# cyrillefavreau/Sol-R

Hardware: AMD Instinct MI355X
Metric: Mrays/s @1920x1080, 3-bounce Cornell (higher is better)
Workload: dtype f32; 1 GPU; cornell 1920x1080, 3 bounces + shadow rays, 75 boxes / 29 primitives, one GPU, whole frame; rays_per_frame=6518779, closest_hit_walks_rank0=3506171, lane_nodes=206382796, lane_prim_tests=37557299, wave_nodes=3396811, wave_prim_tests=626627, wave_walks=106204, cost_ordered_launch_rank0=True, frames_in_flight=3, setup_frames_before_warmup=48, frames_delivered=9105, order_free_nodes=43, short_ray_lists=1, gather=none (one GPU), strips=equal rows, parallelism=tile1

## Files before the change

sol-r_amd/csrc/engine.h:

```cpp
#ifndef SOLR_ENGINE_H
#define SOLR_ENGINE_H

#include <hip/hip_runtime.h>

#include <atomic>
#include <chrono>
#include <cstdio>
#include <cstdlib>
#include <cstring>
#include <string>
#include <vector>

#include "../../include/solr_hip.h"
#include "renderer.h"
#include "lists_device.h"
#include "list_builders.h"

namespace solreng
{
struct HostProfile
{
    const bool on = getenv("SOLR_HIP_HOST_PROFILE") != nullptr;
    struct Entry
    {
        const char *name;
        double seconds;
        long calls;
    } entries[16] = {};
    int used = 0;
    Entry *find(const char *name)
    {
        for (int i = 0; i < used; ++i)
            if (entries[i].name == name)
                return &entries[i];
        if (used < 16)
        {
            entries[used].name = name;
            return &entries[used++];
        }
        return nullptr;
    }
    void report()
    {
        if (!on)
            return;
        for (int i = 0; i < used; ++i)
            fprintf(stderr, "solr_hip host: %-34s %9.3f us per call over %ld calls\n", entries[i].name,
                    1e6 * entries[i].seconds / (entries[i].calls ? entries[i].calls : 1), entries[i].calls);
        used = 0;
    }
    ~HostProfile() { report(); }
};
extern HostProfile gHostProfile;
struct HostSpan
{
    const char *name;
    std::chrono::steady_clock::time_point t0;
    explicit HostSpan(const char *n) : name(n)
    {
        if (gHostProfile.on)
            t0 = std::chrono::steady_clock::now();
    }
    ~HostSpan()
    {
        if (!gHostProfile.on)
            return;
        if (HostProfile::Entry *e = gHostProfile.find(name))
        {
            e->seconds += std::chrono::duration<double>(std::chrono::steady_clock::now() - t0).count();
            e->calls++;
        }
    }
};

struct PhaseTimer
{
    const bool on = getenv("SOLR_HIP_DEBUG_TIMING") != nullptr;
    std::chrono::steady_clock::time_point last = std::chrono::steady_clock::now();
    void mark(const char *what)
    {
        if (!on)
            return;
        const auto now = std::chrono::steady_clock::now();
        fprintf(stderr, "solr_hip: %-28s %8.2f ms\n", what, std::chrono::duration<double, std::milli>(now - last).count());
        last = now;
    }
};

struct DeviceBuffer
{
    void *ptr = nullptr;
    size_t bytes = 0;
};
inline void release(DeviceBuffer &b)
{
    if (b.ptr)
        (void)hipFree(b.ptr);
    b.ptr = nullptr;
    b.bytes = 0;
}

const int MAX_FLIGHTS = 4;
struct Flight
{
    hipStream_t stream = nullptr;
    DeviceBuffer pp, ids;
    DeviceBuffer image[2];
    int side = 0;
    int copy[2] = {-1, -1};
    DeviceBuffer deepStack;
    DeviceBuffer haloAbove, haloBelow, haloSendTop, haloSendBottom;

    DeviceBuffer &shown() { return image[side]; }
    void forgetCopies()
    {
        copy[0] = copy[1] = -1;
        side = 0;
        solreng::release(image[1]);
    }
    void release()
    {
        for (DeviceBuffer *b : {&pp, &ids, &image[0], &deepStack, &haloAbove, &haloBelow, &haloSendTop, &haloSendBottom})
            solreng::release(*b);
        forgetCopies();
    }
};
struct SharedRing
{
    std::atomic<long> done[64][MAX_FLIGHTS + 2];
    std::atomic<long> consumed;
    long frameBytes, imageStride;
};
struct ImageRing
{
    static const int IMAGE_RING = MAX_FLIGHTS + 2;
    BitmapBuffer *pinnedImage[IMAGE_RING] = {};
    size_t pinnedBytes = 0;
    static const long TICKET_PERIOD = ((long)0x7fffffff / IMAGE_RING / IMAGE_RING - 1) * IMAGE_RING;
    static int ticketOf(long serial, int slot) { return (int)((serial % TICKET_PERIOD) * IMAGE_RING + slot); }
    long imageSerial = 0;
    long slotSerial[IMAGE_RING] = {};
    long shareSeq = 0;
    long slotShareSeq[IMAGE_RING] = {};
    long lastWaitedSeq = 0;
    long sharePublished[IMAGE_RING] = {};
    struct SharedRing *sharedRing = nullptr;
    size_t sharedBytes = 0;
    std::string sharedName;
    int shareRank = 0, shareWorld = 0;
    bool slotOfStrips[IMAGE_RING] = {};
    long lastHandedOut = 0;
    bool copyOnRenderStream = false;
    void release();
};
extern ImageRing gImageRing;
struct CopyLane
{
    hipStream_t stream = nullptr;
    hipEvent_t frameRendered = nullptr;
    hipEvent_t imageDone[ImageRing::IMAGE_RING] = {};
    void release();
};
struct ImageStreaming
{
    int next = 0;
    bool ids = false;
    bool valid = false;
    const void *bitmap = nullptr;
    unsigned serial = 0;
    long key[3] = {0, 0, 0};
    DeviceBuffer counters;
    StreamPlan plan = {};
    int bands = 0;
    unsigned *hostWords = nullptr;
    hipEvent_t rendered = nullptr;
    long delivered = 0;
    int support = -1;
    void release();
};
const int SORT_PERIOD = 64;

struct TileSchedule
{
    int mode = 1;
    DeviceBuffer cost, costSnapshot;
    DeviceBuffer order[2];
    int orderBuffer = 0;
    hipEvent_t orderEvent = nullptr;
    bool orderWait[MAX_FLIGHTS] = {};
    unsigned *hostStats = nullptr;
    unsigned *hostStatsDev = nullptr;
    long key[6] = {0, 0, 0, 0, 0, 0};
    int frames = 0;
    bool reorder = false;
    bool orderValid = false;
    BandCuts orderCuts = {};
    void reset()
    {
        frames = 0;
        reorder = false;
        orderValid = false;
    }
    void release();
};

enum Variant
{
    VARIANT_AUTOMATIC = 0,
    VARIANT_EXACT_LIST = 3,
    VARIANT_ALL_FEATURES = 4,
    VARIANT_NO_GROUPING = 5,
    VARIANT_NO_ORDER_FREE = 6,
    VARIANT_STACK_IN_LDS = 7,
    VARIANT_REFERENCE_LEAVES = 8,
    VARIANT_AO_FIXED_STRIDE = 9,
    VARIANT_NAN_DEEP_STACK = 10,
    VARIANT_UNSORTED_LISTS = 12,
    VARIANT_NO_BAND_WORDS = 13,
    VARIANT_ZERO_STREAM_COUNTERS = 14,
    VARIANT_NO_LAMP_CUTOFF = 15,
    VARIANT_ALL_TRIPS = 16
};

struct NodeList
{
    int copies, lists;
    explicit NodeList(int copies_ = 1, int lists_ = 1) : copies(copies_), lists(lists_) {}
    std::vector<float4> rows;
    std::vector<int> start, origin;
    int nb = 0;
    unsigned offRows = 0, offLeaf = 0;
    unsigned offStart = 0;
    int ordered = 0;
    bool tight = false;
    std::vector<int> refitLevels;

    void reset() { *this = NodeList(copies, lists); }
    unsigned nodes() const { return (unsigned)lists * (unsigned)nb; }
    unsigned rowsOf(int list) const { return solrdev::listRows(offRows, (unsigned)nb, (unsigned)list); }
    unsigned offThin() const { return solrdev::listThin(offRows, nodes()); }
    unsigned offSorted() const { return solrdev::listSorted(offRows, nodes()); }
    unsigned layRows(unsigned row)
    {
        offRows = row;
        return row + (unsigned)copies * solrdev::listCopyRows(nodes());
    }
    unsigned layStart(unsigned row)
    {
        offStart = row * 4;
        return row + (nodes() + 3u) / 4u;
    }
    unsigned layLeaf(unsigned row)
    {
        row = (row + 3u) & ~3u;
        offLeaf = row;
        return row + 4u * nodes() + 4u;
    }
};


struct Arena
{
    DeviceBuffer geometry;
    unsigned offPrims = 0, offLights = 0;
    unsigned rowsFixed = 0;
    bool geometryDirty = true;
    bool deviceAhead = false;
    void layOutAgain() { geometryDirty = true; }
};
struct OrderFreeState
{
    int freeCountdown = 0;
    bool freeHostValid = true;
    bool freeDirty = false;
    SolrDeviceLists freeStage;
    bool freeStale = false;
    bool sortedFree = false;
    void dropStage(bool originToo)
    {
        if (freeStage.rows)
            (void)hipFree(freeStage.rows);
        if (freeStage.start)
            (void)hipFree(freeStage.start);
        freeStage.rows = nullptr;
        freeStage.start = nullptr;
        if (originToo && freeStage.origin)
        {
            (void)hipFree(freeStage.origin);
            freeStage.origin = nullptr;
        }
    }
};
struct Rotation
{
    DeviceBuffer movable, refitPlan;
    DeviceBuffer enclosesFlag;
    int nbMovable = -1;
    bool refitReady = false;
    bool refitPlanPending = false;
    bool exactStale = false;
    float exactStaleViewDistance = 0.f;
    int nbDeviceRotations = 0;
};
struct Scene
{
    NodeList exact = NodeList(1, 1), walk = NodeList(2, 1), orderFree = NodeList(3, solrdev::ORDER_FREE_LISTS);
    std::vector<float4> hostPrims;
    int nbPrimitives = 0;
    DeviceBuffer lamps;
    int nbLamps = 0;
    int nested = 1;
    bool walkEncloses = false;
    OrderFreeState lists;
    Rotation rotation;
    Arena arena;

    void newGeometry(int nested_, bool walkEncloses_, int freeCountdown_)
    {
        nested = nested_;
        walkEncloses = walkEncloses_;
        rotation.refitReady = false;
        rotation.exactStale = false;
        rotation.refitPlanPending = true;
        rotation.nbMovable = -1;
        arena.deviceAhead = false;
        orderFree.reset();
        lists.freeCountdown = freeCountdown_;
        lists.freeHostValid = true;
        lists.freeDirty = false;
        lists.dropStage(true);
        lists.freeStale = false;
    }
    bool orderFreeDue() { return lists.freeCountdown > 0 && --lists.freeCountdown == 0; }
    void orderFreeAskAgain() { lists.freeCountdown = 1; }
    void orderFreeBuilt(const NodeList &built, bool stayed, bool fromArena)
    {
        orderFree = built;
        lists.freeHostValid = !stayed;
        lists.freeStale = false;
        rotation.refitReady = false;
        rotation.refitPlanPending = true;
        if (stayed && fromArena)
            lists.freeDirty = true;
        else
            arena.layOutAgain();
    }
    void listsAppended()
    {
        lists.dropStage(false);
        lists.freeDirty = false;
    }
    void arenaFlushed()
    {
        arena.geometryDirty = false;
        lists.freeDirty = false;
    }
    void hostListsPulled()
    {
        lists.freeHostValid = true;
        lists.dropStage(true);
    }
    void hostImagesPulled() { arena.deviceAhead = false; }
    void rotationQueued(bool listsFollow, float viewDistance)
    {
        if (!listsFollow)
            lists.freeStale = orderFree.nb > 0;
        rotation.exactStale = true;
        rotation.exactStaleViewDistance = viewDistance;
    }
    void exactRefitted() { rotation.exactStale = false; }
    void rotationServed(bool walkHolds, bool landed)
    {
        walkEncloses = walkHolds;
        if (landed)
        {
            arena.deviceAhead = true;
            ++rotation.nbDeviceRotations;
        }
    }
    void release()
    {
        lists.dropStage(true);
        for (DeviceBuffer *b : {&arena.geometry, &lamps, &rotation.movable, &rotation.refitPlan, &rotation.enclosesFlag})
            solreng::release(*b);
        *this = Scene();
    }
};
struct Lights
{
    std::vector<float4> hostLights;
    int nbLights = 0;
};
struct TextureUse
{
    int material;
    long texels;
    long offsets[7];
};
struct Materials
{
    DeviceBuffer table;
    unsigned offMatCold = 0;
    int nbMaterials = 0;
    std::vector<int> materialTags;
    std::vector<float> materialAverage;
    std::vector<TextureUse> textureUses;
    void release()
    {
        solreng::release(table);
        *this = Materials();
    }
};
struct Textures
{
    DeviceBuffer atlas;
    size_t atlasBytes = 0;
    bool textureTablesChecked = false;
    void release()
    {
        solreng::release(atlas);
        *this = Textures();
    }
};
struct Randoms
{
    DeviceBuffer values;
    long nbRandoms = 0;
    float randomsReach = 0.f;
    void release()
    {
        solreng::release(values);
        *this = Randoms();
    }
};
struct SceneFacts
{
    bool primsContained = false;
    bool opaqueShadows = false;
    bool plainPlanes = false;
    float sceneExtent = 1.f;
    int sceneFeatures = F_ALL & ~F_FULL;
};
struct KernelTimer
{
    unsigned timingTick = 0;
    std::vector<std::pair<hipEvent_t, hipEvent_t>> events;
    double timedMs = 0.0;
    int timedLaunches = 0;
    std::vector<float> kernelSamples, intervalSamples;
};
struct WalkRecording
{
    DeviceBuffer walkRecords, walkVisits;
    bool recordNext = false;
    bool recorded = false;
    unsigned recordGrid = 0;
    size_t recordLds = 0;
    int recordVariant = -1;
    bool recordDeep = false;
    SceneArgs recordScene = {};
    void release()
    {
        solreng::release(walkRecords);
        solreng::release(walkVisits);
        *this = WalkRecording();
    }
};

struct Engine
{
    bool initialized = false;
    int device = 0;
    int errorCode = 0;
    std::string errorText;

    int variant = VARIANT_AUTOMATIC;
    bool grouping = true;
    int shortRayListsMode = -1;
    int flights = 1;
    bool tileClocks = false;
    int timing = 0;

    Scene scene;
    Lights lights;
    Materials materials;
    Textures textures;
    Randoms randoms;
    SceneFacts facts;

    DeviceBuffer counters, tileClock;
    DeviceBuffer haloGivenAbove, haloGivenBelow;
    int haloSuppliedAbove = 0, haloSuppliedBelow = 0;
    int haloWanted = -1;
    Flight flight[MAX_FLIGHTS];
    bool ownStream = false;
    bool callerStreams = false;
    int current = 0;
    unsigned frameSerial = 0;
    TileSchedule sched;
    unsigned lastSerial = 0;
    int nbTilesTimed = 0;
    void *boundBitmap = nullptr;
    int width = 0, height = 0;
    int firstRow = 0, nbRows = -1;
    int allocW = 0, allocRows = 0;

    KernelTimer timer;
    WalkRecording recording;

    CopyLane copyLane;
    ImageStreaming streaming;
    int tileCheckedX = 0, tileCheckedTiles = 0, tileCheckedShift = 0;
    unsigned tileCheckedMagic = 0;
    int lastMask = -1;
    int lastFrame[6] = {-1, -1, 0, 0, 0, 0};
};

extern Engine gFirst;
extern Engine *gEngines[SOLR_MAX_GPU_COUNT];
extern int gDevices;
extern int gRequested;
extern Engine *gCurrent;
#define g (*gCurrent)
template <class F>
void onEveryDevice(F &&f)
{
    for (int d = 0; d < gDevices; ++d)
    {
        gCurrent = gEngines[d];
        if (gDevices > 1)
            (void)hipSetDevice(g.device);
        f(d);
    }
    gCurrent = &gFirst;
    if (gDevices > 1)
        (void)hipSetDevice(g.device);
}

inline int activeFlights()
{
    if (g.flights < 2 || !(g.ownStream || g.callerStreams))
        return 1;
    int n = 1;
    while (n < g.flights && n < MAX_FLIGHTS && g.flight[n].stream)
        ++n;
    return n;
}
inline bool twoFlights() { return activeFlights() > 1; }
inline hipStream_t sceneStream() { return g.flight[0].stream; }
inline void quiesce()
{
    for (int f = 1; f < MAX_FLIGHTS; ++f)
        if (g.flight[f].stream)
            (void)hipStreamSynchronize(g.flight[f].stream);
    if (g.flight[0].stream)
        (void)hipStreamSynchronize(g.flight[0].stream);
    if (g.copyLane.stream)
        (void)hipStreamSynchronize(g.copyLane.stream);
}

inline void setError(int code, const char *what, const char *file, int line)
{
    if (g.errorCode != 0)
        return;
    g.errorCode = code;
    char buf[512];
    snprintf(buf, sizeof(buf), "%s (%s:%d)", what, file, line);
    g.errorText = buf;
    fprintf(stderr, "solr_hip: error %d: %s\n", code, buf);
    const char *fatal = getenv("SOLR_HIP_FATAL");
    if (fatal && fatal[0] == '1')
        exit(EXIT_FAILURE);
}

#define HIPCHECK(expr)                                                                                           \
    do                                                                                                           \
    {                                                                                                            \
        hipError_t e_ = (expr);                                                                                  \
        if (e_ != hipSuccess)                                                                                    \
        {                                                                                                        \
            std::string m_ = std::string(#expr) + ": " + hipGetErrorString(e_);                                  \
            setError((int)e_, m_.c_str(), __FILE__, __LINE__);                                                   \
        }                                                                                                        \
    } while (0)

#define ARGCHECK(cond, msg)                                                                                      \
    do                                                                                                           \
    {                                                                                                            \
        if (!(cond))                                                                                             \
            setError(-1, msg, __FILE__, __LINE__);                                                               \
    } while (0)

inline bool ok()
{
    return g.errorCode == 0;
}

inline bool ready(const char *who)
{
    if (!ok())
        return false;
    if (!g.initialized)
    {
        setError(-1, (std::string(who) + ": initialize_scene has not been called").c_str(), __FILE__, __LINE__);
        return false;
    }
    return true;
}

inline void reserve(DeviceBuffer &b, size_t bytes)
{
    if (bytes < 16)
        bytes = 16;
    if (b.ptr && b.bytes >= bytes)
        return;
    release(b);
    HIPCHECK(hipMalloc(&b.ptr, bytes));
    if (ok())
        b.bytes = bytes;
}

template <class T>
void upload(DeviceBuffer &b, const std::vector<T> &host)
{
    reserve(b, host.size() * sizeof(T));
    if (ok() && !host.empty())
    {
        HIPCHECK(hipMemcpyAsync(b.ptr, host.data(), host.size() * sizeof(T), hipMemcpyHostToDevice, sceneStream()));
        HIPCHECK(hipStreamSynchronize(sceneStream()));
    }
}

inline int stripRows()
{
    return g.nbRows >= 0 ? g.nbRows : g.height;
}


void h2dSceneOne(BoundingBox *boundingBoxes, int nbActiveBoxes, Primitive *primitives, int nbPrimitives, Lamp *lamps, int nbLamps);
void h2dMaterialsOne(Material *materials, int nbActiveMaterials);
void h2dRandomsOne(float *randoms);
void h2dRandomsSizedOne(const float *randoms, long count);
void h2dTexturesOne(int activeTextures, TextureInfo *textureInfos);
void h2dLightInformationOne(LightInformation *lightInformation, int lightInformationSize);
void setMovableOne(const unsigned char *flags, int nbPrimitives);
void checkTextureTables();
void maybeBuildOrderFreeLists();
void flushGeometry();
void pullGeometry();
void ensureHostFreeLists();
void buildLeafRecords();
bool listEnclosesInArena(const NodeList &list);
ListKnobs listKnobs();
PruneDecider pruneDecider();
bool orderFreeListsUsable();
bool lampCutoffUsable();
bool shortRayListsChoice();
SceneArgs prepareScene(const SceneInfo &sceneInfo, bool exactNodes);
bool deepNodeList(const SceneArgs &S);
bool canRotateOne(const float center[3], const float cosAngles[3], const float sinAngles[3], float viewDistance);
int rotatePrimitivesOne(const float center[3], const float cosAngles[3], const float sinAngles[3], float viewDistance);
void refreshExactList();
void allocateFrame();
int neededFeatures(const SceneInfo &sceneInfo, bool full);
void renderImpl(const SceneInfo &sceneInfo, const vec4i &objects, const PostProcessingInfo &ppInfo, const float origin[3],
                const float direction[3], const float angles[4], bool counting, unsigned long long counts[8]);
void collectEvents();
void d2hBitmapOne(const SceneInfo &sceneInfo, BitmapBuffer *bitmap, PrimitiveXYIdBuffer *primitivesXYIds, bool wait);
void d2hBitmapWait();
void releaseCopies();
bool imageStreamingCuts(int tileRows, int firstRow[SOLR_STREAM_BANDS_MAX + 1], int *bands, bool withIds);
bool armImageStreaming(FrameArgs &F, int tileRows, hipStream_t stream, bool withIds);
void markStreamedFrame(hipStream_t stream);
void ensureCopyStream();
bool ensureImageRing();
int nextTicket(int *slot);
bool haveCommunicator();
bool communicatorUp();
int agreedHaloRows(const PostProcessingInfo &ppInfo);
void exchangeDepthHalo(int flight, hipStream_t stream, const PixelRecord *pp, int W, int firstRow, int nbRows, int frameRows,
                       int wanted, DepthHalo *halo);
bool shareRandoms();

struct HaloDebt
{
    bool owed = false;
    int wanted = 0, width = 0, frameRows = 0;
    ~HaloDebt()
    {
        if (owed)
            exchangeDepthHalo(g.current, g.flight[g.current].stream, nullptr, width, 0, 0, frameRows, wanted, nullptr);
    }
};
void launchPostProcess(const SceneInfo &sceneInfo, const PostProcessingInfo &ppInfo, int flight, hipStream_t stream, int firstRow,
                       int nbRows, unsigned char *bitmap, HaloDebt &debt);
}

namespace solrpost
{
void defaultConversion(hipStream_t stream, const SceneInfo &si, int nbPixels, const PixelRecord *pp, unsigned char *bitmap);
void ambientOcclusion(hipStream_t stream, const SceneInfo &si, const PostProcessingInfo &ppi, int nbRows, const PixelRecord *pp,
                      const float *randoms, long nbRandoms, unsigned char *bitmap, const DepthHalo &halo, int firstRow,
                      float randomsReach, bool heavyFirst);
void depthOfField(hipStream_t stream, const SceneInfo &si, const PostProcessingInfo &ppi, int nbRows, const PixelRecord *pp,
                  const float *randoms, long nbRandoms, unsigned char *bitmap);
void radiosity(hipStream_t stream, const SceneInfo &si, const PostProcessingInfo &ppi, int nbRows, const PixelRecord *pp,
               const int4 *ids, const float *randoms, long nbRandoms, unsigned char *bitmap);
void filter(hipStream_t stream, const SceneInfo &si, const PostProcessingInfo &ppi, int nbRows, const PixelRecord *pp,
            unsigned char *bitmap);
void cartoon(hipStream_t stream, const SceneInfo &si, const PostProcessingInfo &ppi, int nbRows, const PixelRecord *pp,
             unsigned char *bitmap);
void orderTiles(hipStream_t stream, const unsigned *cost, unsigned *snapshot, unsigned *order, int nbTiles,
                volatile unsigned *hostStats, int flights, const BandCuts &cuts);
void packDepthRows(hipStream_t stream, const PixelRecord *pp, int W, int row0, int n, float *out);
}

#endif
```

sol-r_amd/csrc/list_builders.cpp:

```cpp
#include "list_builders.h"

#include <algorithm>
#include <cmath>

namespace solreng
{
int validateNesting(const BoundingBox *boxes, int n)
{
    std::vector<int> ends;
    for (int i = 0; i < n; ++i)
    {
        const int skip = boxes[i].indexForNextBox.x;
        if (skip < 1 || (long)i + skip > n)
            return 0;
        while (!ends.empty() && ends.back() <= i)
            ends.pop_back();
        const int end = i + skip;
        if (!ends.empty() && end > ends.back())
            return 0;
        ends.push_back(end);
    }
    return 1;
}

int collapseChains(const std::vector<float4> &rows, const std::vector<int> &start, bool nested, std::vector<float4> &outRows,
                   std::vector<int> &outStart, std::vector<int> &outOrigin, int *orderedExact, int *orderedWalk)
{
    const int n = (int)start.size();
    auto countOf = [&](int i) { return bitsi(rows[2 * i + 1].z); };
    auto skipOf = [&](int i) { return bitsi(rows[2 * i + 1].w); };
    std::vector<char> keep(n, 1);
    std::vector<int> newIndex((size_t)n + 1);
    newIndex[0] = 0;
    *orderedExact = 1;
    *orderedWalk = 1;
    for (int i = 0; i < n; ++i)
    {
        if (nested && countOf(i) == 0)
        {
            if (i + 1 < n)
            {
                if (skipOf(i) >= 2 && skipOf(i + 1) == skipOf(i) - 1 && memcmp(&rows[2 * i], &rows[2 * i + 2], 16) == 0 &&
                    memcmp(&rows[2 * i + 1], &rows[2 * i + 3], 8) == 0)
                    keep[i] = 0;
            }
            if (skipOf(i) == 1)
                keep[i] = 0;
        }
        const float lo[3] = {rows[2 * i].x, rows[2 * i].y, rows[2 * i].z}, hi[3] = {rows[2 * i + 1].x, rows[2 * i + 1].y, rows[2 * i].w};
        bool ordered = true;
        for (int k = 0; k < 3; ++k)
            ordered = ordered && (lo[k] <= hi[k]) && (fabsf(lo[k]) < 1.0e30f) && (fabsf(hi[k]) < 1.0e30f);
        if (!ordered)
        {
            *orderedExact = 0;
            if (keep[i])
                *orderedWalk = 0;
        }
        newIndex[(size_t)i + 1] = newIndex[i] + (keep[i] ? 1 : 0);
    }
    const int nc = newIndex[n];
    outRows.assign(2 * (size_t)nc, make_float4(0.f, 0.f, 0.f, 0.f));
    outStart.assign(nc, 0);
    outOrigin.assign(nc, 0);
    for (int i = 0; i < n; ++i)
        if (keep[i])
        {
            const int j = newIndex[i];
            outOrigin[j] = i;
            const int end = std::min(i + skipOf(i), n);
            outRows[2 * j] = rows[2 * i];
            outRows[2 * j + 1] = rows[2 * i + 1];
            outRows[2 * j + 1].w = bitsf(newIndex[end] - j);
            outStart[j] = start[i];
        }
    return nc;
}

int pruneInnerNodes(std::vector<float4> &rows, std::vector<int> &start, std::vector<int> &origin, int *nbPruned, double threshold,
                    const PruneDecider &decider)
{
    const int n = (int)start.size();
    *nbPruned = 0;
    if (n < 2 || !(threshold > 0.0))
        return n;
    auto skipOf = [&](int i) { return std::max(bitsi(rows[2 * i + 1].w), 1); };
    auto countOf = [&](int i) { return bitsi(rows[2 * i + 1].z); };
    auto lo = [&](int i, int k) { return k == 0 ? rows[2 * i].x : (k == 1 ? rows[2 * i].y : rows[2 * i].z); };
    auto hi = [&](int i, int k) { return k == 0 ? rows[2 * i + 1].x : (k == 1 ? rows[2 * i + 1].y : rows[2 * i].w); };
    auto areaOf = [&](int i) {
        const double x = (double)hi(i, 0) - lo(i, 0), y = (double)hi(i, 1) - lo(i, 1), z = (double)hi(i, 2) - lo(i, 2);
        return x * y + y * z + z * x;
    };
    std::vector<char> keep(n, 1);
    const int decided = decider ? decider(rows.data(), n, threshold, keep) : -1;
    if (decided >= 0)
        *nbPruned = decided;
    else
    {
        keep.assign(n, 1);
        std::vector<int> leaves;
        std::vector<int> leavesBefore(n + 1, 0);
        for (int i = 0; i < n; ++i)
        {
            leavesBefore[i + 1] = leavesBefore[i] + (countOf(i) > 0 ? 1 : 0);
            if (countOf(i) > 0)
                leaves.push_back(i);
        }
        struct Open
        {
            int node, end;
        };
        std::vector<Open> open;
        double sceneLo[3] = {1e300, 1e300, 1e300}, sceneHi[3] = {-1e300, -1e300, -1e300};
        for (int j = 0; j < n; j += skipOf(j))
            for (int k = 0; k < 3; ++k)
            {
                sceneLo[k] = std::min(sceneLo[k], (double)lo(j, k));
                sceneHi[k] = std::max(sceneHi[k], (double)hi(j, k));
            }
        const double sceneArea = (sceneHi[0] - sceneLo[0]) * (sceneHi[1] - sceneLo[1]) + (sceneHi[1] - sceneLo[1]) * (sceneHi[2] - sceneLo[2]) +
                                 (sceneHi[2] - sceneLo[2]) * (sceneHi[0] - sceneLo[0]);
        for (int i = 0; i < n; ++i)
        {
            while (!open.empty() && open.back().end <= i)
                open.pop_back();
            const int end = std::min(i + skipOf(i), n);
            if (countOf(i) == 0 && end > i + 1)
            {
                const int parentFrom = open.empty() ? 0 : open.back().node, parentTo = open.empty() ? n : open.back().end;
                const double parentArea = open.empty() ? sceneArea : areaOf(open.back().node);
                const double bySurface = parentArea > 0.0 ? std::min(1.0, areaOf(i) / parentArea) : 1.0;
                const int firstLeaf = leavesBefore[parentFrom], lastLeaf = leavesBefore[parentTo];
                const int stride = std::max(1, (lastLeaf - firstLeaf) / 4096);
                int sampled = 0, inside = 0;
                for (int q = firstLeaf; q < lastLeaf; q += stride)
                {
                    const int leaf = leaves[q];
                    bool in = true;
                    for (int k = 0; k < 3 && in; ++k)
                    {
                        const double c = 0.5 * ((double)lo(leaf, k) + hi(leaf, k));
                        in = c >= lo(i, k) && c <= hi(i, k);
                    }
                    ++sampled;
                    inside += in ? 1 : 0;
                }
                const double byOrigin = sampled ? (double)inside / sampled : 1.0;
                bool encloses = true;
                for (int j = i + 1; j < end && encloses; j += skipOf(j))
                    for (int k = 0; k < 3; ++k)
                        encloses = encloses && lo(j, k) >= lo(i, k) && hi(j, k) <= hi(i, k);
                if (encloses && (1.0 - std::max(bySurface, byOrigin)) * (end - i - 1) < threshold)
                {
                    keep[i] = 0;
                    ++*nbPruned;
                    continue;
                }
            }
            open.push_back({i, end});
        }
    }
    if (*nbPruned == 0)
        return n;
    std::vector<int> newIndex(n + 1, 0);
    for (int i = 0; i < n; ++i)
        newIndex[i + 1] = newIndex[i] + (keep[i] ? 1 : 0);
    const int m = newIndex[n];
    std::vector<float4> outRows(2 * (size_t)m);
    std::vector<int> outStart(m), outOrigin(m);
    for (int i = 0; i < n; ++i)
        if (keep[i])
        {
            const int j = newIndex[i];
            const int end = std::min(i + skipOf(i), n);
            outRows[2 * j] = rows[2 * i];
            outRows[2 * j + 1] = rows[2 * i + 1];
            outRows[2 * j + 1].w = bitsf(newIndex[end] - j);
            outStart[j] = start[i];
            outOrigin[j] = origin[i];
        }
    rows.swap(outRows);
    start.swap(outStart);
    origin.swap(outOrigin);
    return m;
}

int groupSiblings(std::vector<float4> &rows, std::vector<int> &start, std::vector<int> &origin, const ListKnobs &knobs)
{
    const int n = (int)start.size();
    auto skipOf = [&](int i) { return bitsi(rows[2 * i + 1].w); };
    struct Bounds
    {
        float lo[3], hi[3];
    };
    auto boundsOf = [&](int i) {
        Bounds b;
        b.lo[0] = rows[2 * i].x, b.lo[1] = rows[2 * i].y, b.lo[2] = rows[2 * i].z;
        b.hi[0] = rows[2 * i + 1].x, b.hi[1] = rows[2 * i + 1].y, b.hi[2] = rows[2 * i].w;
        return b;
    };
    auto merge = [](Bounds a, const Bounds &b) {
        for (int k = 0; k < 3; ++k)
        {
            a.lo[k] = std::min(a.lo[k], b.lo[k]);
            a.hi[k] = std::max(a.hi[k], b.hi[k]);
        }
        return a;
    };
    auto area = [](const Bounds &b) {
        const double x = (double)b.hi[0] - b.lo[0], y = (double)b.hi[1] - b.lo[1], z = (double)b.hi[2] - b.lo[2];
        return x * y + y * z + z * x;
    };
    std::vector<float4> outRows;
    std::vector<int> outStart, outOrigin;
    outRows.reserve(rows.size() + rows.size() / 2);
    outStart.reserve(start.size() + start.size() / 2);
    outOrigin.reserve(start.size() + start.size() / 2);

    std::vector<Bounds> suffix;
    auto splitPoint = [&](const std::vector<int> &sib, int from, int to) {
        const int count = to - from;
        suffix.resize((size_t)count);
        Bounds acc = boundsOf(sib[to - 1]);
        suffix[count - 1] = acc;
        for (int k = count - 2; k >= 0; --k)
        {
            acc = merge(acc, boundsOf(sib[from + k]));
            suffix[k] = acc;
        }
        Bounds left = boundsOf(sib[from]);
        double best = 1e300;
        int bestAt = from + count / 2;
        for (int k = 1; k < count; ++k)
        {
            const double cost = area(left) * k + area(suffix[k]) * (count - k);
            if (cost < best)
            {
                best = cost;
                bestAt = from + k;
            }
            left = merge(left, boundsOf(sib[from + k]));
        }
        return bestAt;
    };

    const int flatMax = std::max(1, knobs.groupFlat);
    struct Emit
    {
        std::function<void(const std::vector<int> &, int, int)> siblings;
        std::function<void(int)> node;
    } emit;
    emit.node = [&](int i) {
        const size_t at = outStart.size();
        outRows.push_back(rows[2 * i]);
        outRows.push_back(rows[2 * i + 1]);
        outStart.push_back(start[i]);
        outOrigin.push_back(origin[i]);
        const int end = std::min(i + skipOf(i), n);
        int few = 0;
        for (int j = i + 1; j < end && few <= flatMax; j += std::max(skipOf(j), 1))
            ++few;
        if (few > flatMax)
        {
            std::vector<int> children;
            for (int j = i + 1; j < end; j += std::max(skipOf(j), 1))
                children.push_back(j);
            emit.siblings(children, 0, (int)children.size());
        }
        else
            for (int j = i + 1; j < end;)
            {
                const int next = j + std::max(skipOf(j), 1);
                emit.node(j);
                j = next;
            }
        outRows[2 * at + 1].w = bitsf((int)(outStart.size() - at));
    };
    const int levels = std::min(4, std::max(1, knobs.groupLevels >= 0 ? knobs.groupLevels : (n <= 64 ? 3 : 2)));
    emit.siblings = [&](const std::vector<int> &sib, int from, int to) {
        if (to - from <= flatMax)
        {
            for (int k = from; k < to; ++k)
                emit.node(sib[k]);
            return;
        }
        {
            Bounds u = boundsOf(sib[from]);
            for (int k = from + 1; k < to; ++k)
                u = merge(u, boundsOf(sib[k]));
            const double limit = 0.5 * area(u);
            bool dominant = false;
            for (int k = from; k < to && !dominant; ++k)
                dominant = area(boundsOf(sib[k])) > limit;
            if (dominant)
            {
                int runStart = from;
                for (int k = from; k <= to; ++k)
                    if (k == to || area(boundsOf(sib[k])) > limit)
                    {
                        if (k > runStart)
                            emit.siblings(sib, runStart, k);
                        if (k < to)
                            emit.node(sib[k]);
                        runStart = k + 1;
                    }
                return;
            }
        }
        int parts[17];
        int np = 1;
        parts[0] = from;
        parts[1] = to;
        for (int level = 0; level < levels; ++level)
        {
            int next[17];
            int nn = 0;
            for (int q = 0; q < np; ++q)
            {
                next[nn++] = parts[q];
                if (parts[q + 1] - parts[q] > 2)
                    next[nn++] = splitPoint(sib, parts[q], parts[q + 1]);
            }
            next[nn] = to;
            np = nn;
            for (int q = 0; q <= np; ++q)
                parts[q] = next[q];
        }
        for (int q = 0; q < np; ++q)
        {
            const int a = parts[q], b = parts[q + 1];
            if (b - a == 1)
            {
                emit.node(sib[a]);
                continue;
            }
            Bounds u = boundsOf(sib[a]);
            for (int k = a + 1; k < b; ++k)
                u = merge(u, boundsOf(sib[k]));
            const size_t at = outStart.size();
            outRows.push_back(make_float4(u.lo[0], u.lo[1], u.lo[2], u.hi[2]));
            outRows.push_back(make_float4(u.hi[0], u.hi[1], bitsf(0), bitsf(1)));
            outStart.push_back(0);
            outOrigin.push_back(-1);
            emit.siblings(sib, a, b);
            outRows[2 * at + 1].w = bitsf((int)(outStart.size() - at));
        }
    };
    std::vector<int> top;
    for (int j = 0; j < n; j += std::max(skipOf(j), 1))
        top.push_back(j);
    emit.siblings(top, 0, (int)top.size());
    rows.swap(outRows);
    start.swap(outStart);
    origin.swap(outOrigin);
    return (int)start.size();
}

int buildWalkOrderList(std::vector<float4> &rows, std::vector<int> &start, std::vector<int> &origin, const ListKnobs &knobs,
                       const PruneDecider &decider, int *prunedBefore, int *prunedAfter, const std::function<void(const char *)> &mark)
{
    pruneInnerNodes(rows, start, origin, prunedBefore, knobs.pruneThreshold, decider);
    if (mark)
        mark("prune");
    groupSiblings(rows, start, origin, knobs);
    if (mark)
        mark("grouping");
    const int n = pruneInnerNodes(rows, start, origin, prunedAfter, knobs.pruneThreshold, decider);
    if (mark)
        mark("prune groups");
    return n;
}

int buildFreeOrderLists(const std::vector<float4> &rows, const std::vector<int> &start, const std::vector<int> &origin,
                        std::vector<float4> &outRows, std::vector<int> &outStart, std::vector<int> &outOrigin, int *nbPruned,
                        double threshold, const PruneDecider &decider)
{
    struct Leaf
    {
        float lo[3], hi[3];
        int node;
    };
    struct TreeNode
    {
        float lo[3], hi[3];
        int left, right, axis, leaf;
        bool keep;
    };
    const int n = (int)start.size();
    std::vector<Leaf> leaves;
    for (int i = 0; i < n; ++i)
        if (bitsi(rows[2 * i + 1].z) > 0)
        {
            Leaf l;
            l.lo[0] = rows[2 * i].x, l.lo[1] = rows[2 * i].y, l.lo[2] = rows[2 * i].z;
            l.hi[0] = rows[2 * i + 1].x, l.hi[1] = rows[2 * i + 1].y, l.hi[2] = rows[2 * i].w;
            l.node = i;
            leaves.push_back(l);
        }
    outRows.clear();
    outStart.clear();
    outOrigin.clear();
    *nbPruned = 0;
    if (leaves.size() < 2)
        return 0;
    auto area = [](const float *lo, const float *hi) {
        const double x = (double)hi[0] - lo[0], y = (double)hi[1] - lo[1], z = (double)hi[2] - lo[2];
        return x * y + y * z + z * x;
    };
    std::vector<TreeNode> tree;
    tree.reserve(2 * leaves.size());
    struct Range
    {
        int from, to, node;
    };
    std::vector<Range> todo;
    tree.push_back(TreeNode());
    todo.push_back({0, (int)leaves.size(), 0});
    while (!todo.empty())
    {
        const Range r = todo.back();
        todo.pop_back();
        const int count = r.to - r.from;
        TreeNode t;
        t.left = t.right = -1;
        t.axis = 0;
        t.leaf = -1;
        t.keep = true;
        if (count == 1)
        {
            for (int k = 0; k < 3; ++k)
                t.lo[k] = leaves[r.from].lo[k], t.hi[k] = leaves[r.from].hi[k];
            t.leaf = leaves[r.from].node;
            tree[r.node] = t;
            continue;
        }
        float clo[3] = {1e30f, 1e30f, 1e30f}, chi[3] = {-1e30f, -1e30f, -1e30f};
        for (int k = 0; k < 3; ++k)
            t.lo[k] = 1e30f, t.hi[k] = -1e30f;
        for (int q = r.from; q < r.to; ++q)
            for (int k = 0; k < 3; ++k)
            {
                t.lo[k] = std::min(t.lo[k], leaves[q].lo[k]);
                t.hi[k] = std::max(t.hi[k], leaves[q].hi[k]);
                const float c = 0.5f * (leaves[q].lo[k] + leaves[q].hi[k]);
                clo[k] = std::min(clo[k], c);
                chi[k] = std::max(chi[k], c);
            }
        for (int k = 0; k < 3; ++k)
            t.lo[k] += 0.f, t.hi[k] += 0.f;
        const int BINS = 16;
        int bestAxis = -1, bestBin = 0;
        double bestCost = 1e300;
        {
            int counts[3][BINS];
            float blo[3][BINS][3], bhi[3][BINS][3];
            float scale[3];
            for (int axis = 0; axis < 3; ++axis)
            {
                const float extent = chi[axis] - clo[axis];
                scale[axis] = extent > 0.f ? BINS / extent : 0.f;
                for (int b = 0; b < BINS; ++b)
                {
                    counts[axis][b] = 0;
                    for (int k = 0; k < 3; ++k)
                        blo[axis][b][k] = 1e30f, bhi[axis][b][k] = -1e30f;
                }
            }
            for (int q = r.from; q < r.to; ++q)
            {
                const Leaf &l = leaves[q];
                for (int axis = 0; axis < 3; ++axis)
                {
                    if (!(scale[axis] > 0.f))
                        continue;
                    const float c = 0.5f * (l.lo[axis] + l.hi[axis]);
                    const int b = std::min(BINS - 1, std::max(0, (int)((c - clo[axis]) * scale[axis])));
                    ++counts[axis][b];
                    float *lo3 = blo[axis][b], *hi3 = bhi[axis][b];
                    lo3[0] = std::min(lo3[0], l.lo[0]), lo3[1] = std::min(lo3[1], l.lo[1]), lo3[2] = std::min(lo3[2], l.lo[2]);
                    hi3[0] = std::max(hi3[0], l.hi[0]), hi3[1] = std::max(hi3[1], l.hi[1]), hi3[2] = std::max(hi3[2], l.hi[2]);
                }
            }
            for (int axis = 0; axis < 3; ++axis)
            {
                if (!(scale[axis] > 0.f))
                    continue;
                double rightArea[BINS];
                int rightCount[BINS];
                float rlo[3] = {1e30f, 1e30f, 1e30f}, rhi[3] = {-1e30f, -1e30f, -1e30f};
                int rc = 0;
                for (int b = BINS - 1; b > 0; --b)
                {
                    rc += counts[axis][b];
                    for (int k = 0; k < 3; ++k)
                    {
                        rlo[k] = std::min(rlo[k], blo[axis][b][k]);
                        rhi[k] = std::max(rhi[k], bhi[axis][b][k]);
                    }
                    rightCount[b] = rc;
                    rightArea[b] = rc ? area(rlo, rhi) : 0.0;
                }
                float llo[3] = {1e30f, 1e30f, 1e30f}, lhi[3] = {-1e30f, -1e30f, -1e30f};
                int lc = 0;
                for (int b = 0; b + 1 < BINS; ++b)
                {
                    lc += counts[axis][b];
                    for (int k = 0; k < 3; ++k)
                    {
                        llo[k] = std::min(llo[k], blo[axis][b][k]);
                        lhi[k] = std::max(lhi[k], bhi[axis][b][k]);
                    }
                    if (lc == 0 || rightCount[b + 1] == 0)
                        continue;
                    const double cost = area(llo, lhi) * lc + rightArea[b + 1] * rightCount[b + 1];
                    if (cost < bestCost)
                    {
                        bestCost = cost;
                        bestAxis = axis;
                        bestBin = b;
                    }
                }
            }
        }
        int mid;
        if (bestAxis < 0)
            mid = r.from + count / 2;
        else
        {
            const float scale = BINS / (chi[bestAxis] - clo[bestAxis]);
            const float origin = clo[bestAxis];
            const int axis = bestAxis, bin = bestBin;
            mid = (int)(std::stable_partition(leaves.begin() + r.from, leaves.begin() + r.to,
                                       [&](const Leaf &l) {
                                           const float c = 0.5f * (l.lo[axis] + l.hi[axis]);
                                           return std::min(BINS - 1, std::max(0, (int)((c - origin) * scale))) <= bin;
                                       }) -
                        leaves.begin());
            if (mid == r.from || mid == r.to)
                mid = r.from + count / 2;
            t.axis = bestAxis;
        }
        t.left = (int)tree.size();
        t.right = t.left + 1;
        tree.push_back(TreeNode());
        tree.push_back(TreeNode());
        tree[r.node] = t;
        todo.push_back({r.from, mid, t.left});
        todo.push_back({mid, r.to, t.right});
    }

    auto flatten = [&](int octant, std::vector<float4> &fr, std::vector<int> &fs, std::vector<int> *which,
                       std::vector<int> *from) {
        struct Visit
        {
            int node, slot;
        };
        std::vector<Visit> stack;
        stack.push_back({0, -1});
        while (!stack.empty())
        {
            const Visit v = stack.back();
            stack.pop_back();
            if (v.slot >= 0)
            {
                fr[2 * v.slot + 1].w = bitsf((int)fs.size() - v.slot);
                continue;
            }
            const TreeNode &t = tree[v.node];
            if (t.leaf >= 0)
            {
                fr.push_back(rows[2 * t.leaf]);
                float4 second = rows[2 * t.leaf + 1];
                second.w = bitsf(1);
                fr.push_back(second);
                fs.push_back(start[t.leaf]);
                if (which)
                    which->push_back(v.node);
                if (from)
                    from->push_back(origin[t.leaf]);
                continue;
            }
            if (t.keep)
            {
                const int slot = (int)fs.size();
                fr.push_back(make_float4(t.lo[0], t.lo[1], t.lo[2], t.hi[2]));
                fr.push_back(make_float4(t.hi[0], t.hi[1], bitsf(0), bitsf(1)));
                fs.push_back(0);
                if (which)
                    which->push_back(v.node);
                if (from)
                    from->push_back(-1);
                stack.push_back({0, slot});
            }
            const bool highFirst = (octant >> t.axis) & 1;
            stack.push_back({highFirst ? t.left : t.right, -1});
            stack.push_back({highFirst ? t.right : t.left, -1});
        }
    };
    {
        std::vector<float4> fr;
        std::vector<int> fs, which;
        flatten(0, fr, fs, &which, nullptr);
        std::vector<int> survivors(which);
        pruneInnerNodes(fr, fs, survivors, nbPruned, threshold, decider);
        std::vector<char> kept(tree.size(), 0);
        for (int t : survivors)
            kept[t] = 1;
        for (size_t t = 0; t < tree.size(); ++t)
            if (tree[t].leaf < 0)
                tree[t].keep = kept[t] != 0;
    }
    std::vector<int> size(tree.size(), 0);
    for (int t = (int)tree.size() - 1; t >= 0; --t)
        size[t] = tree[t].leaf >= 0 ? 1 : (tree[t].keep ? 1 : 0) + size[tree[t].left] + size[tree[t].right];
    const int count = size[0];
    outRows.assign(16 * (size_t)count, make_float4(0.f, 0.f, 0.f, 0.f));
    outStart.assign(8 * (size_t)count, 0);
    outOrigin.assign(8 * (size_t)count, -1);
    struct Place
    {
        int node, at;
    };
    std::vector<Place> stack;
    for (int octant = 0; octant < 8; ++octant)
    {
        float4 *fr = outRows.data() + 2 * (size_t)octant * count;
        int *fs = outStart.data() + (size_t)octant * count, *fo = outOrigin.data() + (size_t)octant * count;
        stack.clear();
        stack.push_back({0, 0});
        while (!stack.empty())
        {
            const Place v = stack.back();
            stack.pop_back();
            const TreeNode &t = tree[v.node];
            if (t.leaf >= 0)
            {
                fr[2 * v.at] = rows[2 * t.leaf];
                float4 second = rows[2 * t.leaf + 1];
                second.w = bitsf(1);
                fr[2 * v.at + 1] = second;
                fs[v.at] = start[t.leaf];
                fo[v.at] = origin[t.leaf];
                continue;
            }
            int at = v.at;
            if (t.keep)
            {
                fr[2 * at] = make_float4(t.lo[0], t.lo[1], t.lo[2], t.hi[2]);
                fr[2 * at + 1] = make_float4(t.hi[0], t.hi[1], bitsf(0), bitsf(size[v.node]));
                ++at;
            }
            const bool highFirst = (octant >> t.axis) & 1;
            const int first = highFirst ? t.right : t.left, second = highFirst ? t.left : t.right;
            stack.push_back({second, at + size[first]});
            stack.push_back({first, at});
        }
    }
    return count;
}

bool listEnclosesOnHost(const std::vector<float4> &rows, const std::vector<int> &start, const std::vector<float4> &prims)
{
    const int n = (int)start.size();
    if (rows.size() < 2 * (size_t)n)
        return false;
    auto skipOf = [&](int i) { return std::max(bitsi(rows[2 * i + 1].w), 1); };
    bool encloses = true;
    for (int i = 0; i < n && encloses; ++i)
    {
        const int end = std::min(i + skipOf(i), n);
        if (bitsi(rows[2 * i + 1].z) > 0 || end <= i + 1)
            continue;
        for (int j = i + 1; j < end && encloses; j += skipOf(j))
            encloses = rows[2 * j].x >= rows[2 * i].x && rows[2 * j].y >= rows[2 * i].y && rows[2 * j].z >= rows[2 * i].z &&
                       rows[2 * j + 1].x <= rows[2 * i + 1].x && rows[2 * j + 1].y <= rows[2 * i + 1].y &&
                       rows[2 * j].w <= rows[2 * i].w;
    }
    const size_t nbPrims = prims.size() / LB_PRIM_ROWS;
    for (int i = 0; i < n && encloses; ++i)
    {
        const int count = bitsi(rows[2 * i + 1].z);
        for (int k = 0; k < count && encloses; ++k)
        {
            const size_t pi = (size_t)start[i] + k;
            if (start[i] < 0 || pi >= nbPrims)
            {
                encloses = false;
                break;
            }
            const float4 *r = &prims[LB_PRIM_ROWS * pi];
            const int type = bitsi(r[LB_ROW_P0_TYPE].w) & LB_PRIM_TYPE_MASK;
            float lo[3] = {r[LB_ROW_P0_TYPE].x, r[LB_ROW_P0_TYPE].y, r[LB_ROW_P0_TYPE].z};
            float hi[3] = {lo[0], lo[1], lo[2]};
            auto add = [&](const float4 &v) {
                lo[0] = std::min(lo[0], v.x), lo[1] = std::min(lo[1], v.y), lo[2] = std::min(lo[2], v.z);
                hi[0] = std::max(hi[0], v.x), hi[1] = std::max(hi[1], v.y), hi[2] = std::max(hi[2], v.z);
            };
            float grow[3] = {r[LB_ROW_SIZE_MAT].x, r[LB_ROW_SIZE_MAT].y, r[LB_ROW_SIZE_MAT].z};
            if (type == ptTriangle)
            {
                add(r[LB_ROW_P1_INDEX]);
                add(r[LB_ROW_P2]);
                grow[0] = grow[1] = grow[2] = 0.f;
            }
            else if (type == ptCylinder)
            {
                add(r[LB_ROW_P1_INDEX]);
                grow[1] = grow[2] = grow[0];
            }
            else if (type == ptSphere)
                grow[1] = grow[2] = grow[0];
            auto slack = [&](int k) { return 4.f * 1.1920929e-7f * std::max(std::max(fabsf(lo[k]), fabsf(hi[k])), fabsf(grow[k])); };
            const float ex = slack(0), ey = slack(1), ez = slack(2);
            encloses = rows[2 * i].x <= lo[0] - fabsf(grow[0]) + ex && rows[2 * i].y <= lo[1] - fabsf(grow[1]) + ey &&
                       rows[2 * i].z <= lo[2] - fabsf(grow[2]) + ez && rows[2 * i + 1].x >= hi[0] + fabsf(grow[0]) - ex &&
                       rows[2 * i + 1].y >= hi[1] + fabsf(grow[1]) - ey && rows[2 * i].w >= hi[2] + fabsf(grow[2]) - ez;
        }
    }
    return encloses;
}

void planRefit(const std::vector<float4> &exact, const std::vector<float4> &walk, const std::vector<int> &origin,
               const std::vector<float4> &free, const std::vector<int> &freeOrigin, std::vector<int> &plan,
               std::vector<int> &exactLevels, std::vector<int> &walkLevels, std::vector<int> &freeLevels)
{
    plan.clear();
    exactLevels.clear();
    walkLevels.clear();
    freeLevels.clear();

    auto heights = [](const std::vector<float4> &rows, std::vector<int> &height) {
        const int n = (int)(rows.size() / 2);
        height.assign(n, 0);
        std::vector<int> parent(n, -1), stack;
        for (int i = 0; i < n; ++i)
        {
            while (!stack.empty() && i >= stack.back() + std::max(bitsi(rows[2 * stack.back() + 1].w), 1))
                stack.pop_back();
            parent[i] = stack.empty() ? -1 : stack.back();
            stack.push_back(i);
        }
        int top = 0;
        for (int i = n - 1; i >= 0; --i)
        {
            if (parent[i] >= 0)
                height[parent[i]] = std::max(height[parent[i]], height[i] + 1);
            top = std::max(top, height[i]);
        }
        return n ? top + 1 : 0;
    };
    auto byHeight = [&](const std::vector<int> &height, int nbHeights, std::vector<int> &levels, auto entry) {
        std::vector<std::vector<int>> bucket((size_t)nbHeights);
        for (int i = 0; i < (int)height.size(); ++i)
        {
            const long e = entry(i);
            if (e != -1)
                bucket[(size_t)height[i]].push_back((int)e);
        }
        for (const std::vector<int> &b : bucket)
            if (!b.empty())
            {
                levels.push_back((int)plan.size());
                levels.push_back((int)b.size());
                plan.insert(plan.end(), b.begin(), b.end());
            }
    };
    std::vector<int> height;
    int nbHeights = heights(exact, height);
    byHeight(height, nbHeights, exactLevels, [](int i) { return i != 0 ? (long)i : -1L; });
    nbHeights = heights(walk, height);
    byHeight(height, nbHeights, walkLevels, [&](int j) {
        if (origin[j] == 0)
            return -1L;
        return origin[j] < 0 ? (long)(j | (int)0x80000000) : (long)j;
    });
    if (!free.empty())
    {
        nbHeights = heights(free, height);
        byHeight(height, nbHeights, freeLevels, [&](int j) {
            if (freeOrigin[j] == 0)
                return -1L;
            return freeOrigin[j] < 0 ? (long)(j | (int)0x80000000) : (long)j;
        });
    }
    if (plan.empty())
        plan.push_back(0);
}
}
```

sol-r_amd/csrc/list_builders.h:

```cpp
#ifndef SOLR_LIST_BUILDERS_H
#define SOLR_LIST_BUILDERS_H

#include <hip/hip_vector_types.h>

#include <cstring>
#include <functional>
#include <vector>

#include "../../include/solr_types.h"

namespace solreng
{
inline int bitsi(float v)
{
    int i;
    memcpy(&i, &v, sizeof(i));
    return i;
}
inline float bitsf(int v)
{
    float f;
    memcpy(&f, &v, 4);
    return f;
}

enum ListBuilderPrimRow
{
    LB_ROW_P0_TYPE = 0,
    LB_ROW_SIZE_MAT = 1,
    LB_ROW_P1_INDEX = 2,
    LB_ROW_P2 = 3,
    LB_PRIM_ROWS = 8,
    LB_PRIM_TYPE_MASK = 0xff
};

struct ListKnobs
{
    double pruneThreshold = 1.0;
    int groupFlat = 4;
    int groupLevels = -1;
};

typedef std::function<int(const float4 *rows, int n, double threshold, std::vector<char> &keep)> PruneDecider;

int validateNesting(const BoundingBox *boxes, int n);
int collapseChains(const std::vector<float4> &rows, const std::vector<int> &start, bool nested, std::vector<float4> &outRows,
                   std::vector<int> &outStart, std::vector<int> &outOrigin, int *orderedExact, int *orderedWalk);
int pruneInnerNodes(std::vector<float4> &rows, std::vector<int> &start, std::vector<int> &origin, int *nbPruned, double threshold,
                    const PruneDecider &decider = nullptr);
int groupSiblings(std::vector<float4> &rows, std::vector<int> &start, std::vector<int> &origin, const ListKnobs &knobs);
int buildWalkOrderList(std::vector<float4> &rows, std::vector<int> &start, std::vector<int> &origin, const ListKnobs &knobs,
                       const PruneDecider &decider, int *prunedBefore, int *prunedAfter,
                       const std::function<void(const char *)> &mark = nullptr);
int buildFreeOrderLists(const std::vector<float4> &rows, const std::vector<int> &start, const std::vector<int> &origin,
                        std::vector<float4> &outRows, std::vector<int> &outStart, std::vector<int> &outOrigin, int *nbPruned,
                        double threshold, const PruneDecider &decider = nullptr);
bool listEnclosesOnHost(const std::vector<float4> &rows, const std::vector<int> &start, const std::vector<float4> &prims);
void planRefit(const std::vector<float4> &exact, const std::vector<float4> &walk, const std::vector<int> &origin,
               const std::vector<float4> &free, const std::vector<int> &freeOrigin, std::vector<int> &plan,
               std::vector<int> &exactLevels, std::vector<int> &walkLevels, std::vector<int> &freeLevels);
}

#endif
```

sol-r_amd/csrc/lists_device.h:

```cpp
#pragma once
#include <hip/hip_runtime.h>

#include <vector>

struct SolrDeviceLists
{
    float4 *rows = nullptr;
    int *start = nullptr;
    int *origin = nullptr;
};

int solrBuildOrderFreeListsOnDevice(const float4 *rows, const int *start, const int *origin, int n, double threshold,
                                    int *nbPruned, hipStream_t stream, SolrDeviceLists *stay);

int solrPruneDecisionsOnDevice(const float4 *rows, int n, double threshold, std::vector<char> &keep, hipStream_t stream);
```

sol-r_amd/csrc/solr_arena.hip:

```cpp
#include <hip/hip_runtime.h>

#include <cmath>

#include "../../include/solr_hip.h"
#include "rt_device.h"

using namespace solrdev;

#include "renderer.h"
#include "engine.h"

using namespace solreng;

namespace solreng
{
__global__ __launch_bounds__(256) void k_buildLeafRecords(float4 *__restrict__ arena, unsigned offNodes, unsigned offStart,
                                                         unsigned offPrims, unsigned offLeaf, int nbNodes)
{
    const int i = blockIdx.x * blockDim.x + threadIdx.x;
    if (i >= nbNodes)
        return;
    float4 r0 = make_float4(0.f, 0.f, 0.f, 0.f), r1 = r0, r2 = r0, r3 = r0;
    const int nb = __float_as_int(arena[offNodes + 2u * (unsigned)i + 1u].z);
    if (nb > 0)
    {
        const int start = ((const int *)arena)[offStart + (unsigned)i];
        const float4 *prim = arena + offPrims + 8u * (unsigned)start;
        r0 = prim[ROW_P0_TYPE];
        r1 = prim[ROW_SIZE_MAT];
        r2 = prim[ROW_P1_INDEX];
        r3 = prim[ROW_P2];
        if (planeClass(__float_as_int(r0.w) & PRIM_TYPE_MASK))
        {
            const float4 n0 = prim[ROW_N0];
            r2 = make_float4(n0.x, n0.y, n0.z, r2.w);
            r3 = make_float4(r3.w, 0.f, 0.f, 0.f);
        }
        r3.w = __int_as_float(start);
    }
    float4 *out = arena + offLeaf + 4u * (unsigned)i;
    out[0] = r0;
    out[1] = r1;
    out[2] = r2;
    out[3] = r3;
}

__global__ __launch_bounds__(256) void k_tightenLeaves(float4 *__restrict__ arena, unsigned offNodes, unsigned offTight,
                                                      unsigned offStart, unsigned offPrims, int nbNodes, float margin)
{
    const int i = blockIdx.x * blockDim.x + threadIdx.x;
    if (i >= nbNodes)
        return;
    float4 row0 = arena[offNodes + 2u * (unsigned)i], row1 = arena[offNodes + 2u * (unsigned)i + 1u];
    const int nb = __float_as_int(row1.z);
    if (nb > 0)
    {
        const int start = ((const int *)arena)[offStart + (unsigned)i];
        float lx = INFINITY, ly = INFINITY, lz = INFINITY, hx = -INFINITY, hy = -INFINITY, hz = -INFINITY;
        bool plain = true;
        for (int k = 0; k < nb && plain; ++k)
        {
            const float4 *prim = arena + offPrims + 8u * (unsigned)(start + k);
            const float4 p = prim[ROW_P0_TYPE], s = prim[ROW_SIZE_MAT];
            const int kind = (__float_as_int(p.w) >> PRIM_KIND_SHIFT) & 15;
            plain = kind == KIND_PLANE_XY || kind == KIND_PLANE_YZ || kind == KIND_PLANE_XZ;
            const float ex = kind == KIND_PLANE_YZ ? margin : fabsf(s.x) + margin;
            const float ey = kind == KIND_PLANE_XZ ? margin : fabsf(s.y) + margin;
            const float ez = kind == KIND_PLANE_XY ? margin : fabsf(s.z) + margin;
            lx = fminf(lx, p.x - ex), hx = fmaxf(hx, p.x + ex);
            ly = fminf(ly, p.y - ey), hy = fmaxf(hy, p.y + ey);
            lz = fminf(lz, p.z - ez), hz = fmaxf(hz, p.z + ez);
        }
        plain = plain && lx <= hx && ly <= hy && lz <= hz && fabsf(lx) < 3.0e38f && fabsf(hx) < 3.0e38f && fabsf(ly) < 3.0e38f &&
                fabsf(hy) < 3.0e38f && fabsf(lz) < 3.0e38f && fabsf(hz) < 3.0e38f;
        if (plain)
        {
            const float nlx = fmaxf(row0.x, lx), nly = fmaxf(row0.y, ly), nlz = fmaxf(row0.z, lz);
            const float nhx = fminf(row1.x, hx), nhy = fminf(row1.y, hy), nhz = fminf(row0.w, hz);
            if (nlx <= nhx && nly <= nhy && nlz <= nhz)
            {
                row0 = make_float4(nlx, nly, nlz, nhz);
                row1 = make_float4(nhx, nhy, row1.z, row1.w);
            }
        }
    }
    arena[offTight + 2u * (unsigned)i] = row0;
    arena[offTight + 2u * (unsigned)i + 1u] = row1;
}

__global__ __launch_bounds__(256) void k_tightenInner(float4 *__restrict__ arena, unsigned offTight, int nbNodes, int listLength)
{
    const int i = blockIdx.x * blockDim.x + threadIdx.x;
    if (i >= nbNodes)
        return;
    const float4 row0 = arena[offTight + 2u * (unsigned)i], row1 = arena[offTight + 2u * (unsigned)i + 1u];
    const int nb = __float_as_int(row1.z), skip = __float_as_int(row1.w);
    if (nb > 0 || skip <= 1)
        return;
    const int listEnd = (i / listLength + 1) * listLength;
    const int end = min(i + skip, listEnd);
    float lx = INFINITY, ly = INFINITY, lz = INFINITY, hx = -INFINITY, hy = -INFINITY, hz = -INFINITY;
    for (int j = i + 1; j < end; ++j)
    {
        const float4 b = arena[offTight + 2u * (unsigned)j + 1u];
        if (__float_as_int(b.z) <= 0)
            continue;
        const float4 a = arena[offTight + 2u * (unsigned)j];
        lx = fminf(lx, a.x), ly = fminf(ly, a.y), lz = fminf(lz, a.z);
        hx = fmaxf(hx, b.x), hy = fmaxf(hy, b.y), hz = fmaxf(hz, a.w);
    }
    const float nlx = fmaxf(row0.x, lx), nly = fmaxf(row0.y, ly), nlz = fmaxf(row0.z, lz);
    const float nhx = fminf(row1.x, hx), nhy = fminf(row1.y, hy), nhz = fminf(row0.w, hz);
    if (!(nlx <= nhx && nly <= nhy && nlz <= nhz))
        return;
    arena[offTight + 2u * (unsigned)i] = make_float4(nlx, nly, nlz, nhz);
    arena[offTight + 2u * (unsigned)i + 1u] = make_float4(nhx, nhy, row1.z, row1.w);
}

__global__ __launch_bounds__(256) void k_listEncloses(const float4 *__restrict__ arena, unsigned offNodes, unsigned offStart,
                                                      unsigned offPrims, int nbNodes, int nbPrims, int *bad)
{
    const int i = blockIdx.x * blockDim.x + threadIdx.x;
    if (i >= nbNodes)
        return;
    const float4 a = arena[offNodes + 2u * (unsigned)i], b = arena[offNodes + 2u * (unsigned)i + 1u];
    const int count = __float_as_int(b.z);
    const int end = min(i + max(__float_as_int(b.w), 1), nbNodes);
    bool encloses = true;
    if (count <= 0)
    {
        for (int j = i + 1; j < end && encloses;)
        {
            const float4 ca = arena[offNodes + 2u * (unsigned)j], cb = arena[offNodes + 2u * (unsigned)j + 1u];
            encloses = ca.x >= a.x && ca.y >= a.y && ca.z >= a.z && cb.x <= b.x && cb.y <= b.y && ca.w <= a.w;
            j += max(__float_as_int(cb.w), 1);
        }
    }
    else
    {
        const int start = ((const int *)arena)[offStart + (unsigned)i];
        for (int k = 0; k < count && encloses; ++k)
        {
            const long long pi = (long long)start + k;
            if (start < 0 || pi >= nbPrims)
            {
                encloses = false;
                break;
            }
            const float4 *r = arena + offPrims + (size_t)PRIM_ROWS * (size_t)pi;
            const float4 p0 = r[ROW_P0_TYPE], size = r[ROW_SIZE_MAT];
            const int type = __float_as_int(p0.w) & PRIM_TYPE_MASK;
            float lo[3] = {p0.x, p0.y, p0.z}, hi[3] = {p0.x, p0.y, p0.z};
            auto add = [&](const float4 &v) {
                lo[0] = v.x < lo[0] ? v.x : lo[0], lo[1] = v.y < lo[1] ? v.y : lo[1], lo[2] = v.z < lo[2] ? v.z : lo[2];
                hi[0] = hi[0] < v.x ? v.x : hi[0], hi[1] = hi[1] < v.y ? v.y : hi[1], hi[2] = hi[2] < v.z ? v.z : hi[2];
            };
            float grow[3] = {size.x, size.y, size.z};
            if (type == ptTriangle)
            {
                add(r[ROW_P1_INDEX]);
                add(r[ROW_P2]);
                grow[0] = grow[1] = grow[2] = 0.f;
            }
            else if (type == ptCylinder)
            {
                add(r[ROW_P1_INDEX]);
                grow[1] = grow[2] = grow[0];
            }
            else if (type == ptSphere)
                grow[1] = grow[2] = grow[0];
            auto larger = [](float x, float y) { return x < y ? y : x; };
            auto slack = [&](int k) { return 4.f * 1.1920929e-7f * larger(larger(fabsf(lo[k]), fabsf(hi[k])), fabsf(grow[k])); };
            const float ex = slack(0), ey = slack(1), ez = slack(2);
            encloses = a.x <= lo[0] - fabsf(grow[0]) + ex && a.y <= lo[1] - fabsf(grow[1]) + ey && a.z <= lo[2] - fabsf(grow[2]) + ez &&
                       b.x >= hi[0] + fabsf(grow[0]) - ex && b.y >= hi[1] + fabsf(grow[1]) - ey && a.w >= hi[2] + fabsf(grow[2]) - ez;
        }
    }
    if (!encloses)
        *bad = 1;
}

void ensureHostFreeLists()
{
    if (g.scene.lists.freeHostValid || !ok())
        return;
    quiesce();
    NodeList &list = g.scene.orderFree;
    const size_t n = list.nodes();
    list.rows.resize(2 * n);
    list.start.resize(n);
    list.origin.resize(n);
    const bool staged = g.scene.lists.freeStage.rows != nullptr;
    const char *arena = (const char *)g.scene.arena.geometry.ptr;
    if (!staged && !arena)
    {
        setError(-1, "order-free lists neither staged nor in the arena", __FILE__, __LINE__);
        return;
    }
    HIPCHECK(hipMemcpy(list.rows.data(), staged ? (const void *)g.scene.lists.freeStage.rows : arena + (size_t)list.offRows * 16, 2 * n * 16,
                       hipMemcpyDeviceToHost));
    HIPCHECK(hipMemcpy(list.start.data(), staged ? (const void *)g.scene.lists.freeStage.start : arena + (size_t)list.offStart * 4, n * 4,
                       hipMemcpyDeviceToHost));
    if (g.scene.lists.freeStage.origin)
        HIPCHECK(hipMemcpy(list.origin.data(), g.scene.lists.freeStage.origin, n * 4, hipMemcpyDeviceToHost));
    if (ok())
    {
        g.scene.hostListsPulled();
    }
}

void pullGeometry()
{
    if (!g.scene.arena.deviceAhead || !g.scene.arena.geometry.ptr)
        return;
    refreshExactList();
    quiesce();
    auto get = [&](unsigned at, void *dst, size_t bytes) {
        if (bytes)
            HIPCHECK(hipMemcpy(dst, (const char *)g.scene.arena.geometry.ptr + (size_t)at * 16, bytes, hipMemcpyDeviceToHost));
    };
    for (NodeList *list : {&g.scene.exact, &g.scene.walk, &g.scene.orderFree})
        if (list != &g.scene.orderFree || g.scene.lists.freeHostValid)
            get(list->offRows, list->rows.data(), list->rows.size() * 16);
    get(g.scene.arena.offPrims, g.scene.hostPrims.data(), g.scene.hostPrims.size() * 16);
    g.scene.hostImagesPulled();
}

static bool tightenList(const NodeList &list)
{
    static const bool off = getenv("SOLR_HIP_NO_TIGHT_LEAVES") != nullptr;
    const int nbNodes = (int)list.nodes(), listLength = list.nb;
    if (off || !g.facts.plainPlanes || nbNodes <= 0 || listLength <= 0 || listLength > 65536 || !ok())
        return false;
    float4 *arena = (float4 *)g.scene.arena.geometry.ptr;
    const float margin = g.facts.sceneExtent * (1.f / 1024.f);
    const dim3 grid((unsigned)((nbNodes + 255) / 256));
    hipLaunchKernelGGL(k_tightenLeaves, grid, dim3(256), 0, sceneStream(), arena, list.offRows, list.offThin(), list.offStart, g.scene.arena.offPrims,
                       nbNodes, margin);
    hipLaunchKernelGGL(k_tightenInner, grid, dim3(256), 0, sceneStream(), arena, list.offThin(), nbNodes, listLength);
    HIPCHECK(hipGetLastError());
    return ok();
}

__global__ __launch_bounds__(256) void k_sortNodeBounds(float4 *__restrict__ arena, unsigned offBoxesFree, unsigned offSorted, int nb)
{
    const int i = blockIdx.x * blockDim.x + threadIdx.x;
    if (i > 8 * nb)
        return;
    float4 a = make_float4(0.f, 0.f, 0.f, 0.f), b = a;
    if (i < 8 * nb)
    {
        const int octant = i / nb;
        a = arena[offBoxesFree + 2u * (unsigned)i];
        b = arena[offBoxesFree + 2u * (unsigned)i + 1u];
        if (octant & 1)
        {
            const float t = a.x;
            a.x = b.x;
            b.x = t;
        }
        if (octant & 2)
        {
            const float t = a.y;
            a.y = b.y;
            b.y = t;
        }
        if (octant & 4)
        {
            const float t = a.z;
            a.z = a.w;
            a.w = t;
        }
        b.w = __int_as_float(__float_as_int(b.w) << 5);
    }
    arena[offSorted + 2u * (unsigned)i] = a;
    arena[offSorted + 2u * (unsigned)i + 1u] = b;
}

static bool sortFreeLists()
{
    static const bool off = getenv("SOLR_HIP_NO_SORTED_LISTS") != nullptr;
    const NodeList &list = g.scene.orderFree;
    if (off || list.nb <= 0 || !ok())
        return false;
    hipLaunchKernelGGL(k_sortNodeBounds, dim3((unsigned)((8 * list.nb + 1 + 255) / 256)), dim3(256), 0, sceneStream(),
                       (float4 *)g.scene.arena.geometry.ptr, list.offRows, list.offSorted(), list.nb);
    HIPCHECK(hipGetLastError());
    return ok();
}

static void deriveList(NodeList &list)
{
    const bool orderFree = &list == &g.scene.orderFree;
    const int n = (orderFree && g.scene.lists.freeStale) ? 0 : (int)list.nodes();
    if (n > 0)
        hipLaunchKernelGGL(k_buildLeafRecords, dim3((unsigned)((n + 255) / 256)), dim3(256), 0, sceneStream(), (float4 *)g.scene.arena.geometry.ptr,
                           list.offRows, list.offStart, g.scene.arena.offPrims, list.offLeaf, n);
    HIPCHECK(hipGetLastError());
    list.tight = list.copies > 1 && n > 0 && tightenList(list);
    if (orderFree)
        g.scene.lists.sortedFree = n > 0 && sortFreeLists();
}

void buildLeafRecords()
{
    if (!ok() || !g.scene.arena.geometry.ptr)
        return;
    for (NodeList *list : {&g.scene.exact, &g.scene.walk, &g.scene.orderFree})
        deriveList(*list);
    HIPCHECK(hipStreamSynchronize(sceneStream()));
}

static void copyStagedLists()
{
    const NodeList &list = g.scene.orderFree;
    char *arena = (char *)g.scene.arena.geometry.ptr;
    const SolrDeviceLists &stage = g.scene.lists.freeStage;
    HIPCHECK(hipMemcpyAsync(arena + (size_t)list.offRows * 16, stage.rows, (size_t)list.nodes() * 32, hipMemcpyDeviceToDevice, sceneStream()));
    HIPCHECK(hipMemcpyAsync(arena + (size_t)list.offStart * 4, stage.start, (size_t)list.nodes() * 4, hipMemcpyDeviceToDevice, sceneStream()));
}

static void appendFreeLists()
{
    const unsigned end = g.scene.orderFree.layLeaf(g.scene.orderFree.layStart(g.scene.orderFree.layRows(g.scene.arena.rowsFixed)));
    const size_t bytes = (size_t)end * 16, fixedBytes = (size_t)g.scene.arena.rowsFixed * 16;
    PhaseTimer phase;
    if (g.scene.arena.geometry.bytes < bytes)
    {
        DeviceBuffer larger;
        reserve(larger, bytes);
        if (!ok())
            return;
        HIPCHECK(hipMemcpyAsync(larger.ptr, g.scene.arena.geometry.ptr, fixedBytes, hipMemcpyDeviceToDevice, sceneStream()));
        HIPCHECK(hipStreamSynchronize(sceneStream()));
        release(g.scene.arena.geometry);
        g.scene.arena.geometry = larger;
    }
    HIPCHECK(hipMemsetAsync((char *)g.scene.arena.geometry.ptr + fixedBytes, 0, bytes - fixedBytes, sceneStream()));
    copyStagedLists();
    if (ok())
        deriveList(g.scene.orderFree);
    HIPCHECK(hipStreamSynchronize(sceneStream()));
    phase.mark("geometry: lists appended");
    if (ok())
        g.scene.listsAppended();
}

void flushGeometry()
{
    if (!g.scene.arena.geometryDirty)
    {
        if (g.scene.lists.freeDirty && g.scene.lists.freeStage.rows && g.scene.arena.geometry.ptr && g.scene.arena.rowsFixed > 0)
            appendFreeLists();
        else if (g.scene.lists.freeDirty)
            g.scene.arena.layOutAgain();
        if (!g.scene.arena.geometryDirty)
            return;
    }
    pullGeometry();
    if (!g.scene.lists.freeStage.rows)
        ensureHostFreeLists();
    unsigned row = g.scene.walk.layRows(g.scene.exact.layRows(0));
    row = (row + 3u) & ~3u;
    g.scene.arena.offPrims = row;
    row += (unsigned)g.scene.hostPrims.size();
    g.scene.arena.offLights = row;
    row += (unsigned)g.lights.hostLights.size();
    row = g.scene.walk.layStart(g.scene.exact.layStart(row));
    row = g.scene.walk.layLeaf(g.scene.exact.layLeaf(row));
    g.scene.arena.rowsFixed = row;
    row = g.scene.orderFree.layLeaf(g.scene.orderFree.layStart(g.scene.orderFree.layRows(row)));
    PhaseTimer phase;
    reserve(g.scene.arena.geometry, (size_t)std::max(row, 1u) * 16);
    if (!ok())
        return;
    HIPCHECK(hipMemsetAsync(g.scene.arena.geometry.ptr, 0, (size_t)std::max(row, 1u) * 16, sceneStream()));
    auto put = [&](unsigned at, const void *src, size_t bytes) {
        if (bytes && ok())
            HIPCHECK(hipMemcpyAsync((char *)g.scene.arena.geometry.ptr + (size_t)at * 16, src, bytes, hipMemcpyHostToDevice, sceneStream()));
    };
    for (const NodeList *list : {&g.scene.exact, &g.scene.walk, &g.scene.orderFree})
        if (list == &g.scene.orderFree && g.scene.lists.freeStage.rows)
        {
            if (ok())
                copyStagedLists();
        }
        else
        {
            put(list->offRows, list->rows.data(), list->rows.size() * 16);
            put(list->offStart / 4, list->start.data(), list->start.size() * 4);
        }
    put(g.scene.arena.offPrims, g.scene.hostPrims.data(), g.scene.hostPrims.size() * 16);
    put(g.scene.arena.offLights, g.lights.hostLights.data(), g.lights.hostLights.size() * 16);
    HIPCHECK(hipStreamSynchronize(sceneStream()));
    if (ok())
        g.scene.lists.dropStage(false);
    phase.mark("geometry: upload");
    buildLeafRecords();
    phase.mark("geometry: leaf records");
    if (ok())
        g.scene.arenaFlushed();
}

bool listEnclosesInArena(const NodeList &list)
{
    const int n = (int)list.nodes();
    HIPCHECK(hipSetDevice(g.device));
    reserve(g.scene.rotation.enclosesFlag, sizeof(int));
    if (!ok())
        return false;
    int found = 1;
    HIPCHECK(hipMemsetAsync(g.scene.rotation.enclosesFlag.ptr, 0, sizeof(int), sceneStream()));
    hipLaunchKernelGGL(k_listEncloses, dim3((unsigned)((n + 255) / 256)), dim3(256), 0, sceneStream(),
                       (const float4 *)g.scene.arena.geometry.ptr, list.offRows, list.offStart, g.scene.arena.offPrims, n,
                       (int)(g.scene.hostPrims.size() / PRIM_ROWS), (int *)g.scene.rotation.enclosesFlag.ptr);
    HIPCHECK(hipGetLastError());
    HIPCHECK(hipMemcpyAsync(&found, g.scene.rotation.enclosesFlag.ptr, sizeof(int), hipMemcpyDeviceToHost, sceneStream()));
    HIPCHECK(hipStreamSynchronize(sceneStream()));
    return ok() && found == 0;
}

ListKnobs listKnobs()
{
    ListKnobs knobs;
    if (const char *v = getenv("SOLR_HIP_PRUNE"))
        knobs.pruneThreshold = atof(v);
    if (const char *v = getenv("SOLR_HIP_GROUP_FLAT"))
        knobs.groupFlat = atoi(v);
    if (const char *v = getenv("SOLR_HIP_GROUP_LEVELS"))
        knobs.groupLevels = std::max(atoi(v), 0);
    return knobs;
}

PruneDecider pruneDecider()
{
    if (getenv("SOLR_HIP_LISTS_ON_HOST"))
        return nullptr;
    const hipStream_t stream = sceneStream();
    return [stream](const float4 *rows, int n, double threshold, std::vector<char> &keep) {
        return solrPruneDecisionsOnDevice(rows, n, threshold, keep, stream);
    };
}

void maybeBuildOrderFreeLists()
{
    if (!g.scene.orderFreeDue())
        return;
    if (!g.facts.primsContained)
    {
        g.scene.orderFreeAskAgain();
        return;
    }
    PhaseTimer phase;
    quiesce();
    pullGeometry();
    if (!ok())
        return;
    phase.mark("order-free: host images");
    const std::vector<float4> &rows = g.scene.exact.rows;
    const std::vector<int> &start = g.scene.exact.start;
    const int n = (int)start.size();
    if (n < 2 || rows.size() != 2 * (size_t)n || n > 16000000)
        return;
    const ListKnobs knobs = listKnobs();
    const bool onHost = getenv("SOLR_HIP_LISTS_ON_HOST") != nullptr;
    const bool fromArena = !g.scene.arena.geometryDirty && g.scene.arena.geometry.ptr != nullptr && !g.scene.rotation.exactStale &&
                           !g.scene.arena.deviceAhead && !onHost;
    const float4 *arena = (const float4 *)g.scene.arena.geometry.ptr;
    const bool encloses = fromArena ? listEnclosesInArena(g.scene.exact) : listEnclosesOnHost(rows, start, g.scene.hostPrims);
    if (!ok())
        return;
    if (!encloses)
    {
        if (getenv("SOLR_HIP_DEBUG_TREE"))
            fprintf(stderr, "solr_hip: no order-free lists: a node does not hold its children or primitives\n");
        return;
    }
    phase.mark("order-free: checks");
    std::vector<int> origin;
    auto ownOrigins = [&]() {
        origin.resize(n);
        for (int i = 0; i < n; ++i)
            origin[i] = i;
    };
    int prunedFree = 0;
    int count = -1;
    if (!onHost)
    {
        HIPCHECK(hipSetDevice(g.device));
        if (ok() && knobs.pruneThreshold > 0.0)
        {
            g.scene.lists.dropStage(true);
            if (fromArena)
                count = solrBuildOrderFreeListsOnDevice(arena + g.scene.exact.offRows, (const int *)arena + g.scene.exact.offStart, nullptr, n,
                                                        knobs.pruneThreshold, &prunedFree, sceneStream(), &g.scene.lists.freeStage);
            else
            {
                ownOrigins();
                count = solrBuildOrderFreeListsOnDevice(rows.data(), start.data(), origin.data(), n, knobs.pruneThreshold, &prunedFree,
                                                        sceneStream(), &g.scene.lists.freeStage);
            }
        }
    }
    const bool stayed = count > 0 && g.scene.lists.freeStage.rows != nullptr;
    NodeList built(g.scene.orderFree.copies, g.scene.orderFree.lists);
    if (count < 0)
    {
        if (origin.empty())
            ownOrigins();
        count = buildFreeOrderLists(rows, start, origin, built.rows, built.start, built.origin, &prunedFree, knobs.pruneThreshold,
                                    pruneDecider());
    }
    if (getenv("SOLR_HIP_DEBUG_TREE"))
        fprintf(stderr, "solr_hip: order-free lists: 8 x %d nodes (%d inner nodes that hardly cull left out)\n", count, prunedFree);
    if (count <= 0)
        return;
    phase.mark("order-free: tree, pruning, eight flattenings");
    built.nb = count;
    g.scene.orderFreeBuilt(built, stayed, fromArena);
}

bool orderFreeListsUsable()
{
    return g.scene.orderFree.nb > 0 && g.facts.primsContained && !g.scene.lists.freeStale && g.scene.nested && g.scene.walk.ordered &&
           g.variant != VARIANT_NO_ORDER_FREE;
}

bool lampCutoffUsable()
{
    return g.scene.walkEncloses && g.facts.primsContained && g.scene.nested && g.scene.walk.ordered && g.variant != VARIANT_NO_LAMP_CUTOFF;
}

static int tightListsFor(const SceneArgs &S, const SceneInfo &sceneInfo, bool exactNodes)
{
    if (exactNodes || g.variant == VARIANT_REFERENCE_LEAVES || !g.scene.walk.tight || !g.scene.walkEncloses || !sceneInfo.extendedGeometry)
        return 0;
    if (S.nbBoxesFree > 0 && !g.scene.orderFree.tight)
        return 0;
    return (sceneInfo.viewDistance > 0.f && sceneInfo.viewDistance <= 64.f * g.facts.sceneExtent) ? 1 : 0;
}

static bool sortedListsUsable(int nbBoxesFree)
{
    return nbBoxesFree > 0 && g.scene.lists.sortedFree && g.variant != VARIANT_UNSORTED_LISTS;
}

bool shortRayListsChoice()
{
    static const int fromEnv = getenv("SOLR_HIP_SHORT_RAY_LISTS") ? atoi(getenv("SOLR_HIP_SHORT_RAY_LISTS")) : -1;
    const int mode = g.shortRayListsMode >= 0 ? g.shortRayListsMode : fromEnv;
    return mode < 0 ? activeFlights() >= 2 : mode != 0;
}

static SceneArgs makeScene(bool exactNodes)
{
    const NodeList &list = exactNodes ? g.scene.exact : g.scene.walk;
    SceneArgs S;
    memset(&S, 0, sizeof(S));
    S.geometry = g.scene.arena.geometry.ptr;
    S.materials = g.materials.table.ptr;
    S.textures = g.textures.atlas.ptr;
    S.randoms = g.randoms.values.ptr;
    S.offBoxes = list.offRows;
    S.offBoxStart = list.offStart;
    S.offLeaf = list.offLeaf;
    S.offPrims = g.scene.arena.offPrims;
    S.offLights = g.scene.arena.offLights;
    S.offMatCold = g.materials.offMatCold;
    S.nbBoxes = list.nb;
    S.nbPrimitives = g.scene.nbPrimitives;
    S.nbLights = g.lights.nbLights;
    S.nbLamps = g.scene.nbLamps;
    S.nested = g.scene.nested;
    S.orderedBoxes = list.ordered;
    S.nbRandoms = g.randoms.values.ptr ? g.randoms.nbRandoms : 0;
    if (!exactNodes && orderFreeListsUsable())
    {
        S.offBoxesFree = g.scene.orderFree.offRows;
        S.offLeafFree = g.scene.orderFree.offLeaf;
        S.nbBoxesFree = g.scene.orderFree.nb;
        S.opaqueShadows = g.facts.opaqueShadows ? SHADOWS_OPAQUE : 0;
        S.shortRayLists = shortRayListsChoice() ? 1 : 0;
    }
    if (!exactNodes && lampCutoffUsable())
        S.opaqueShadows |= SHADOWS_LAMP_CUTOFF;
    if (g.variant == VARIANT_ALL_TRIPS)
        S.opaqueShadows |= SHADOWS_ALL_TRIPS;
    S.tightLists = 0;
    S.sortedLists = sortedListsUsable(S.nbBoxesFree) ? 1 : 0;
    return S;
}

SceneArgs prepareScene(const SceneInfo &sceneInfo, bool exactNodes)
{
    maybeBuildOrderFreeLists();
    flushGeometry();
    if (exactNodes)
        refreshExactList();
    if (!ok())
        return SceneArgs();
    SceneArgs S = makeScene(exactNodes);
    S.tightLists = tightListsFor(S, sceneInfo, exactNodes);
    return S;
}

bool deepNodeList(const SceneArgs &S)
{
    return S.nbBoxes > 1024;
}

}
```

sol-r_amd/csrc/solr_diag.hip:

```cpp
#include <hip/hip_runtime.h>
#include <dlfcn.h>
#include <fcntl.h>
#include <sched.h>
#include <sys/mman.h>
#include <sys/stat.h>
#include <unistd.h>

#include <atomic>

#include <cmath>
#include <cstdio>
#include <cstdlib>
#include <cstring>
#include <string>
#include <functional>
#include <chrono>
#include <vector>

#include "../../include/solr_hip.h"
#include "rt_device.h"
#include "device_pool.h"
#include "lists_device.h"

using namespace solrdev;

#include "renderer.h"
#include "engine.h"

using namespace solreng;

namespace solrprobe
{
int residentScene(const SceneInfo &sceneInfo, bool exactNodes, SceneArgs *S, int *features, int *deepList, hipStream_t *stream)
{
    if (!ready("solr_hip_probe"))
        return -1;
    quiesce();
    HIPCHECK(hipSetDevice(g.device));
    ARGCHECK(g.materials.table.ptr != nullptr, "solr_hip_probe: no materials uploaded");
    if (!ok())
        return -1;
    checkTextureTables();
    *S = prepareScene(sceneInfo, exactNodes);
    if (!ok())
        return -1;
    *features = neededFeatures(sceneInfo, false);
    *deepList = deepNodeList(*S);
    *stream = g.flight[0].stream;
    return 0;
}
void fail(int code, const char *what) { setError(code, what, __FILE__, __LINE__); }

int postProcess(const SceneInfo &sceneInfo, const PostProcessingInfo &ppInfo, const PostProcessingBuffer *frame,
                unsigned char *bitmapOut)
{
    if (!ready("solr_hip_probe_postprocess"))
        return -1;
    quiesce();
    HIPCHECK(hipSetDevice(g.device));
    ARGCHECK(frame != nullptr && bitmapOut != nullptr, "solr_hip_probe_postprocess: no buffer");
    ARGCHECK(sceneInfo.size.x > 0 && sceneInfo.size.y > 0, "solr_hip_probe_postprocess: empty image");
    ARGCHECK(g.nbRows < 0 && gDevices == 1, "solr_hip_probe_postprocess: whole frames of one device only");
    if (!ok())
        return -1;
    g.width = sceneInfo.size.x;
    g.height = sceneInfo.size.y;
    allocateFrame();
    if (!ok())
        return -1;
    const int flight = g.current;
    const hipStream_t stream = g.flight[flight].stream;
    const size_t pixels = (size_t)g.width * g.height;
    HIPCHECK(hipMemcpyAsync(g.flight[flight].pp.ptr, frame, pixels * sizeof(PostProcessingBuffer), hipMemcpyHostToDevice, stream));
    unsigned char *bitmap = (unsigned char *)g.flight[flight].shown().ptr;
    const bool neighbourhood = (ppInfo.type == ppe_ambientOcclusion || ppInfo.type == ppe_depthOfField ||
                                ppInfo.type == ppe_radiosity || ppInfo.type == ppe_filter || ppInfo.type == ppe_cartoon);
    if (neighbourhood)
    {
        HaloDebt nothingOwed;
        launchPostProcess(sceneInfo, ppInfo, flight, stream, 0, g.height, bitmap, nothingOwed);
    }
    else
    {
        solrpost::defaultConversion(stream, sceneInfo, (int)pixels, (const PixelRecord *)g.flight[flight].pp.ptr, bitmap);
        HIPCHECK(hipGetLastError());
    }
    HIPCHECK(hipMemcpyAsync(bitmapOut, bitmap, pixels * SOLR_COLOR_DEPTH, hipMemcpyDeviceToHost, stream));
    HIPCHECK(hipStreamSynchronize(stream));
    return ok() ? 0 : -1;
}

void lastFrame(int out[6])
{
    memcpy(out, g.lastFrame, sizeof(g.lastFrame));
}

int listCopy(int list, int what, void *out, int capacity)
{
    if (!ready("solr_hip_probe_list_copy"))
        return -1;
    ARGCHECK(list >= 0 && list <= 2 && what >= 0 && what <= 4, "solr_hip_probe_list_copy: no such list or copy");
    ARGCHECK(g.scene.arena.geometry.ptr != nullptr || g.scene.arena.geometryDirty, "solr_hip_probe_list_copy: no scene uploaded");
    if (!ok())
        return -1;
    HIPCHECK(hipSetDevice(g.device));
    flushGeometry();
    if (list == 1)
        refreshExactList();
    quiesce();
    if (!ok() || !g.scene.arena.geometry.ptr)
        return -1;
    const NodeList &L = list == 0 ? g.scene.walk : (list == 1 ? g.scene.exact : g.scene.orderFree);
    const unsigned nodes = (list == 2 && g.scene.lists.freeStale) ? 0u : L.nodes();
    size_t at = 0, count = 0, unit = 16;
    switch (what)
    {
    case 0:
        at = (size_t)L.offRows * 16, count = 2 * (size_t)nodes;
        break;
    case 1:
        at = (size_t)L.offThin() * 16, count = (L.copies > 1 && L.tight) ? 2 * (size_t)nodes : 0;
        break;
    case 2:
        at = (size_t)L.offSorted() * 16, count = (list == 2 && L.copies > 2 && g.scene.lists.sortedFree) ? 2 * (size_t)nodes + 2 : 0;
        break;
    case 3:
        at = (size_t)L.offLeaf * 16, count = 4 * (size_t)nodes;
        break;
    default:
        at = (size_t)L.offStart * 4, count = nodes, unit = 4;
        break;
    }
    if (nodes == 0)
        count = 0;
    if (!out)
        return (int)count;
    ARGCHECK(count <= (size_t)(capacity < 0 ? 0 : capacity), "solr_hip_probe_list_copy: capacity too small");
    ARGCHECK(at + count * unit <= g.scene.arena.geometry.bytes, "solr_hip_probe_list_copy: the copy lies outside the arena");
    if (!ok())
        return -1;
    if (count)
        HIPCHECK(hipMemcpy(out, (const char *)g.scene.arena.geometry.ptr + at, count * unit, hipMemcpyDeviceToHost));
    return ok() ? (int)count : -1;
}

int walkOffer(const SceneInfo &sceneInfo, bool exactNodes, int out[8])
{
    SceneArgs S;
    int features, deep;
    hipStream_t stream;
    if (residentScene(sceneInfo, exactNodes, &S, &features, &deep, &stream) != 0)
        return -1;
    const float margin = g.facts.sceneExtent * (1.f / 1024.f), extent = g.facts.sceneExtent;
    out[0] = S.tightLists, out[1] = S.sortedLists, out[2] = S.nbBoxesFree, out[3] = S.opaqueShadows, out[4] = S.shortRayLists;
    out[5] = S.nbBoxes;
    memcpy(&out[6], &margin, 4);
    memcpy(&out[7], &extent, 4);
    return 0;
}
}

extern "C" {
static unsigned long long walkLists[6];
void solr_hip_walk_bound_lists(unsigned long long out[6])
{
    if (out)
        memcpy(out, walkLists, sizeof(walkLists));
}

static int recordFrame(const SceneInfo *sceneInfo, const vec4i *objects, const PostProcessingInfo *postProcessingInfo,
                       const float origin[3], const float direction[3], const float angles[4], const char *who)
{
    quiesce();
    HIPCHECK(hipSetDevice(g.device));
    g.recording.recorded = false;
    g.recording.recordNext = true;
    if (!ok())
        return -1;
    renderImpl(*sceneInfo, *objects, *postProcessingInfo, origin, direction, angles, false, nullptr);
    g.recording.recordNext = false;
    HIPCHECK(hipStreamSynchronize(g.flight[g.current].stream));
    if (!ok() || !g.recording.recorded)
    {
        if (ok())
            setError(-1, "solr_hip_walk_bound: the frame was not recorded", __FILE__, __LINE__);
        return -1;
    }
    (void)who;
    return 0;
}

static int replayRecords(unsigned grid, size_t ldsBytes, int repeats, double ms[3], unsigned long long stats[4], bool lists)
{
    typedef WalkBoundFn BoundFn;
    ARGCHECK(g.recording.recordVariant >= 0 && g.recording.recordVariant < solrrows::LEAN_ROWS && g.recording.walkRecords.ptr && grid > 0 &&
                 (size_t)grid * SOLR_WALK_SLOT_BYTES <= g.recording.walkRecords.bytes,
             "solr_hip_walk_replay: no recorded frame, or more workgroups than its buffer holds");
    if (!ok())
        return -1;
    const int row = g.recording.recordVariant;
    const BoundFn fn = solrrows::walkBound(row, solrrows::ROWS[row].features | (g.recording.recordDeep ? F_DEEP : 0));
    ARGCHECK(fn != nullptr, "solr_hip_walk_bound: no replay instantiation for this row");
    if (!ok())
        return -1;
    reserve(g.recording.walkVisits, (size_t)grid * WAVE * sizeof(unsigned) + 64);
    hipEvent_t e0 = nullptr, e1 = nullptr;
    HIPCHECK(hipEventCreate(&e0));
    HIPCHECK(hipEventCreate(&e1));
    if (!ok())
        return -1;
    const hipStream_t stream = g.flight[g.current].stream;
    unsigned *visits = (unsigned *)g.recording.walkVisits.ptr;
    unsigned *skipped = visits + (size_t)grid * WAVE;
    double sum = 0.0, best = 1.0e30;
    repeats = repeats < 1 ? 1 : repeats;
    for (int i = 0; i < repeats + 2 && ok(); ++i)
    {
        HIPCHECK(hipMemsetAsync(skipped, 0, sizeof(unsigned), stream));
        HIPCHECK(hipEventRecord(e0, stream));
        hipLaunchKernelGGL(fn, dim3(grid), dim3(WAVE), ldsBytes, stream, g.recording.recordScene, (const char *)g.recording.walkRecords.ptr,
                           visits, skipped);
        HIPCHECK(hipGetLastError());
        HIPCHECK(hipEventRecord(e1, stream));
        HIPCHECK(hipEventSynchronize(e1));
        float t = 0.f;
        HIPCHECK(hipEventElapsedTime(&t, e0, e1));
        if (i >= 2)
        {
            sum += t;
            best = t < best ? t : best;
        }
    }
    if (ok() && stats)
    {
        std::vector<unsigned> v((size_t)grid * WAVE + 1);
        HIPCHECK(hipMemcpy(v.data(), visits, v.size() * sizeof(unsigned), hipMemcpyDeviceToHost));
        std::vector<int> heads((size_t)grid * 4);
        HIPCHECK(hipMemcpy2D(heads.data(), 16, g.recording.walkRecords.ptr, SOLR_WALK_SLOT_BYTES, 16, grid, hipMemcpyDeviceToHost));
        if (const char *dump = getenv("SOLR_HIP_WALK_BOUND_DUMP"))
        {
            if (FILE *f = fopen(dump, "wb"))
            {
                const unsigned n = grid;
                fwrite(&n, sizeof(n), 1, f);
                fwrite(v.data(), sizeof(unsigned), (size_t)n * WAVE, f);
                fwrite(heads.data(), sizeof(int), (size_t)n * 4, f);
                fclose(f);
            }
        }
        unsigned long long walks = 0, entries = 0;
        for (unsigned b = 0; b < grid; ++b)
            walks += (unsigned long long)heads[4 * (size_t)b];
        if (lists)
        {
            std::vector<int> kinds((size_t)grid * 4 * (SOLR_WALK_SLOTS + 1));
            HIPCHECK(hipMemcpy2D(kinds.data(), 16 * (SOLR_WALK_SLOTS + 1), g.recording.walkRecords.ptr, SOLR_WALK_SLOT_BYTES,
                                 16 * (SOLR_WALK_SLOTS + 1), grid, hipMemcpyDeviceToHost));
            for (int i = 0; i < 6; ++i)
                walkLists[i] = 0;
            for (unsigned b = 0; ok() && b < grid; ++b)
            {
                const int *slot = &kinds[(size_t)b * 4 * (SOLR_WALK_SLOTS + 1)];
                const int n = std::min(slot[0], (int)SOLR_WALK_SLOTS);
                for (int j = 0; j < n; ++j)
                {
                    const int kind = slot[4 * (1 + j)], freeList = slot[4 * (1 + j) + 1];
                    if (kind == WALK_CLOSEST || kind == WALK_SHADOW)
                        ++walkLists[2 * kind + (freeList ? 1 : 0)];
                    else
                        ++walkLists[4];
                }
                walkLists[5] += (unsigned long long)(slot[0] - n);
            }
        }
        for (size_t i = 0; i + 1 < v.size(); ++i)
            entries += v[i];
        stats[0] = walks;
        stats[1] = v.back();
        stats[2] = entries;
        stats[3] = grid;
    }
    if (ms)
    {
        ms[0] = 0.0;
        ms[1] = sum / repeats;
        ms[2] = best;
    }
    (void)hipEventDestroy(e0);
    (void)hipEventDestroy(e1);
    return ok() ? 0 : -1;
}

static bool keepWalkRecords = false;

int solr_hip_walk_bound(const SceneInfo *sceneInfo, const vec4i *objects, const PostProcessingInfo *postProcessingInfo,
                        const float origin[3], const float direction[3], const float angles[4], int repeats, double ms[3],
                        unsigned long long stats[4])
{
    if (!ready("solr_hip_walk_bound"))
        return -1;
    ARGCHECK(gDevices == 1, "solr_hip_walk_bound: a diagnostic of one engine; this process renders on several devices");
    if (!ok())
        return -1;
    if (recordFrame(sceneInfo, objects, postProcessingInfo, origin, direction, angles, "solr_hip_walk_bound") != 0)
        return -1;
    const int rc = replayRecords(g.recording.recordGrid, g.recording.recordLds, repeats, ms, stats, true);
    if (!keepWalkRecords)
    {
        release(g.recording.walkRecords);
        release(g.recording.walkVisits);
        g.recording.recorded = false;
    }
    return rc;
}

void solr_hip_walk_records_keep(int keep)
{
    keepWalkRecords = keep != 0;
}

int solr_hip_walk_records_info(unsigned long long info[4])
{
    if (!ready("solr_hip_walk_records_info") || !info)
        return -1;
    info[0] = g.recording.recorded ? g.recording.recordGrid : 0;
    info[1] = SOLR_WALK_SLOT_BYTES;
    info[2] = g.recording.recordLds;
    info[3] = SOLR_WALK_SLOTS;
    return 0;
}

int solr_hip_walk_records_copy(void *host, unsigned grid, int toDevice)
{
    if (!ready("solr_hip_walk_records_copy"))
        return -1;
    ARGCHECK(host && grid > 0 && g.recording.recorded, "solr_hip_walk_records_copy: no recorded frame");
    if (!ok())
        return -1;
    const size_t bytes = (size_t)grid * SOLR_WALK_SLOT_BYTES;
    HIPCHECK(hipSetDevice(g.device));
    if (toDevice)
    {
        reserve(g.recording.walkRecords, bytes);
        if (!ok())
            return -1;
        HIPCHECK(hipMemcpy(g.recording.walkRecords.ptr, host, bytes, hipMemcpyHostToDevice));
    }
    else
    {
        ARGCHECK(bytes <= g.recording.walkRecords.bytes, "solr_hip_walk_records_copy: more workgroups than were recorded");
        if (!ok())
            return -1;
        HIPCHECK(hipMemcpy(host, g.recording.walkRecords.ptr, bytes, hipMemcpyDeviceToHost));
    }
    return ok() ? 0 : -1;
}

int solr_hip_walk_replay(unsigned grid, long ldsBytes, int repeats, double ms[3], unsigned long long stats[4])
{
    if (!ready("solr_hip_walk_replay"))
        return -1;
    ARGCHECK(g.recording.recorded, "solr_hip_walk_replay: no recorded frame (solr_hip_walk_records_keep(1), then solr_hip_walk_bound)");
    if (!ok())
        return -1;
    HIPCHECK(hipSetDevice(g.device));
    return replayRecords(grid, ldsBytes < 0 ? g.recording.recordLds : (size_t)ldsBytes, repeats, ms, stats, false);
}

void solr_hip_walk_records_release(void)
{
    release(g.recording.walkRecords);
    release(g.recording.walkVisits);
    g.recording.recorded = false;
}

void solr_hip_enable_timing(int enable)
{
    onEveryDevice([&](int) {
        g.timing = enable > 0 ? enable : 0;
        g.timer.timingTick = 0;
    });
}

void solr_hip_set_frames_in_flight(int n)
{
    onEveryDevice([&](int) {
        quiesce();
        if (g.initialized)
            (void)hipSetDevice(g.device);
        const int before = g.flights;
        g.flights = n < 1 ? 1 : (n > MAX_FLIGHTS ? MAX_FLIGHTS : n);
        g.current = 0;
        if (g.flights != before)
            g.sched.orderValid = false;
        if (g.initialized && g.width > 0)
            allocateFrame();
    });
}

int solr_hip_get_frames_in_flight(void)
{
    return activeFlights();
}

void *solr_hip_flight_stream(int flight)
{
    return (flight >= 0 && flight < MAX_FLIGHTS) ? (void *)g.flight[flight].stream : nullptr;
}

int solr_hip_next_flight(void)
{
    return twoFlights() ? (int)(g.frameSerial % (unsigned)activeFlights()) : 0;
}

void solr_hip_set_tile_scheduling(int mode)
{
    onEveryDevice([&](int) {
        g.sched.mode = mode < 0 ? 0 : (mode > 2 ? 2 : mode);
        g.sched.reset();
    });
}

int solr_hip_split_tiles(void)
{
    return (g.sched.hostStats && g.sched.orderValid) ? (int)g.sched.hostStats[5] : 0;
}

int solr_hip_tile_scheduling_active(void)
{
    return (g.sched.mode == 2 || (g.sched.mode == 1 && g.sched.reorder)) && g.sched.orderValid ? 1 : 0;
}

void solr_hip_enable_tile_clocks(int enable)
{
    g.tileClocks = enable != 0;
}

int solr_hip_tile_clocks(unsigned long long *clocks, int capacityTiles)
{
    if (!g.initialized || !g.tileClock.ptr || !clocks || capacityTiles <= 0)
        return 0;
    const int n = g.nbTilesTimed < capacityTiles ? g.nbTilesTimed : capacityTiles;
    quiesce();
    if (hipMemcpy(clocks, g.tileClock.ptr, (size_t)n * 2 * sizeof(unsigned long long), hipMemcpyDeviceToHost) !=
        hipSuccess)
        return 0;
    return n;
}

double solr_hip_kernel_time(int *nbLaunches, int reset)
{
    if (g.initialized && g.flight[0].stream)
        (void)hipStreamSynchronize(g.flight[0].stream);
    collectEvents();
    double ms = g.timer.timedMs;
    if (nbLaunches)
        *nbLaunches = g.timer.timedLaunches;
    if (reset)
    {
        g.timer.timedMs = 0.0;
        g.timer.timedLaunches = 0;
        g.timer.kernelSamples.clear();
        g.timer.intervalSamples.clear();
    }
    return ms;
}

int solr_hip_timing_samples(float *kernelMs, float *intervalMs, int capacity)
{
    if (g.initialized && g.flight[0].stream)
        (void)hipStreamSynchronize(g.flight[0].stream);
    collectEvents();
    const int n = std::min((int)g.timer.kernelSamples.size(), std::max(capacity, 0));
    for (int i = 0; i < n; ++i)
    {
        if (kernelMs)
            kernelMs[i] = g.timer.kernelSamples[i];
        if (intervalMs)
            intervalMs[i] = g.timer.intervalSamples[i];
    }
    return n;
}

void solr_hip_set_short_ray_lists(int mode)
{
    onEveryDevice([&](int) { g.shortRayListsMode = mode < 0 ? -1 : (mode != 0 ? 1 : 0); });
}

int solr_hip_short_ray_lists(void)
{
    return shortRayListsChoice() ? 1 : 0;
}

void solr_hip_set_variant(int variant)
{
    onEveryDevice([&](int) {
        g.variant = variant;
        g.grouping = (variant != VARIANT_NO_GROUPING);
    });
}

int solr_hip_get_variant(void)
{
    return g.variant;
}

void solr_hip_memory_usage(unsigned long long bytes[4])
{
    bytes[0] = g.scene.arena.geometry.bytes + g.scene.lamps.bytes + g.scene.rotation.movable.bytes + g.scene.rotation.refitPlan.bytes;
    bytes[1] = g.materials.table.bytes;
    bytes[2] = g.textures.atlas.bytes;
    bytes[3] = g.randoms.values.bytes;
    for (const Flight &set : g.flight)
        bytes[3] += set.pp.bytes + set.ids.bytes + set.image[0].bytes + set.deepStack.bytes;
}


extern "C" int solr_hip_order_free_nodes(void)
{
    return (g.initialized && orderFreeListsUsable()) ? g.scene.orderFree.nb : 0;
}

extern "C" int solr_hip_order_free_shadows(void)
{
    return (g.initialized && orderFreeListsUsable() && g.facts.opaqueShadows) ? 1 : 0;
}

extern "C" int solr_hip_shadow_lamp_cutoff(void)
{
    return (g.initialized && lampCutoffUsable()) ? 1 : 0;
}

#ifdef SOLR_TIMING
void solr_hip_wave_cycles(unsigned long long out[16], int reset)
{
    (void)hipDeviceSynchronize();
    std::vector<unsigned long long> slots(16 * SOLR_TIMING_SLOTS);
    (void)hipMemcpy(slots.data(), (unsigned long long *)g.counters.ptr + 16, slots.size() * sizeof(unsigned long long),
                    hipMemcpyDeviceToHost);
    if (out)
        for (int k = 0; k < 16; ++k)
        {
            out[k] = 0;
            for (size_t w = 0; w < SOLR_TIMING_SLOTS; ++w)
                out[k] += slots[16 * w + k];
        }
    if (reset)
        (void)hipMemset((unsigned long long *)g.counters.ptr + 16, 0, slots.size() * sizeof(unsigned long long));
}
int solr_hip_wave_cycle_slots(unsigned long long *out, int capacityWorkgroups)
{
    (void)hipDeviceSynchronize();
    const size_t n = std::min((size_t)std::max(capacityWorkgroups, 0), (size_t)SOLR_TIMING_SLOTS);
    (void)hipMemcpy(out, (unsigned long long *)g.counters.ptr + 16, 16 * n * sizeof(unsigned long long), hipMemcpyDeviceToHost);
    return (int)n;
}
#endif
}
```

sol-r_amd/csrc/solr_lists.hip:

```cpp
#include <hip/hip_runtime.h>
#include <hipcub/hipcub.hpp>

#include <cstdio>
#include <cstdlib>
#include <cstring>
#include <mutex>
#include <vector>

#include <chrono>

#include "device_pool.h"
#include "lists_device.h"

namespace
{
struct Phase
{
    const bool on = getenv("SOLR_HIP_DEBUG_TIMING") != nullptr;
    std::chrono::steady_clock::time_point last = std::chrono::steady_clock::now();
    void mark(const char *what, int detail = -1)
    {
        if (!on)
            return;
        const auto now = std::chrono::steady_clock::now();
        if (detail >= 0)
            fprintf(stderr, "solr_lists: %-24s %8.2f ms (%d)\n", what, std::chrono::duration<double, std::milli>(now - last).count(), detail);
        else
            fprintf(stderr, "solr_lists: %-24s %8.2f ms\n", what, std::chrono::duration<double, std::milli>(now - last).count());
        last = now;
    }
};

const int BINS = 16;
const int MAX_DEPTH = 64;

struct Node
{
    float lo[3], hi[3];
    float clo[3], chi[3];
    int from, to;
    int left, right, axis, bin;
    int leaf;
    int keep;
    int keptAncestor;
    int size;
    int mid;
    int split;
};

struct BinSet
{
    int count[3][BINS];
    float lo[3][BINS][3], hi[3][BINS][3];
};

template <class T>
struct Dev
{
    T *p = nullptr;
    size_t n = 0;
    bool own = false;
    bool alloc(size_t count)
    {
        n = count;
        const size_t bytes = std::max(count, (size_t)1) * sizeof(T);
        p = (T *)solrScratchPool().take(bytes);
        return p != nullptr || allocOwn(count);
    }
    bool allocOwn(size_t count)
    {
        n = count;
        own = true;
        return hipMalloc((void **)&p, std::max(count, (size_t)1) * sizeof(T)) == hipSuccess;
    }
    ~Dev()
    {
        if (p && own)
            (void)hipFree(p);
    }
};

__device__ inline void atomicMinF(float *addr, float v)
{
    v += 0.f;
    if (v >= 0.f)
        atomicMin((int *)addr, __float_as_int(v));
    else
        atomicMax((unsigned *)addr, __float_as_uint(v));
}
__device__ inline void atomicMaxF(float *addr, float v)
{
    v += 0.f;
    if (v >= 0.f)
        atomicMax((int *)addr, __float_as_int(v));
    else
        atomicMin((unsigned *)addr, __float_as_uint(v));
}

__global__ void k_open(Node *nodes, BinSet *bins, int first, int count)
{
    const int i = blockIdx.x * blockDim.x + threadIdx.x;
    if (i >= count)
        return;
    Node &t = nodes[first + i];
    BinSet &b = bins[i];
    for (int axis = 0; axis < 3; ++axis)
        for (int bin = 0; bin < BINS; ++bin)
        {
            b.count[axis][bin] = 0;
            for (int k = 0; k < 3; ++k)
            {
                b.lo[axis][bin][k] = 1e30f;
                b.hi[axis][bin][k] = -1e30f;
            }
        }
    for (int k = 0; k < 3; ++k)
    {
        t.lo[k] = t.clo[k] = 1e30f;
        t.hi[k] = t.chi[k] = -1e30f;
    }
    t.left = t.right = -1;
    t.axis = 0;
    t.bin = 0;
    t.leaf = -1;
    t.keep = 1;
    t.split = 0;
    t.mid = t.from;
}

__device__ inline float waveMin(float v)
{
    for (int off = 32; off > 0; off >>= 1)
        v = fminf(v, __shfl_xor(v, off, 64));
    return v;
}
__device__ inline float waveMax(float v)
{
    for (int off = 32; off > 0; off >>= 1)
        v = fmaxf(v, __shfl_xor(v, off, 64));
    return v;
}

__global__ __launch_bounds__(256) void k_bounds(Node *nodes, const int *nodeOf, const int *order, const float *llo, const float *lhi,
                                                 int nbLeaves, int levelFirst)
{
    const int i = blockIdx.x * blockDim.x + threadIdx.x;
    const int t = i < nbLeaves ? nodeOf[i] : -1;
    const bool open = t >= levelFirst && nodes[t].to - nodes[t].from > 1;
    if (t >= levelFirst && !open)
    {
        Node &node = nodes[t];
        const int leaf = order[i];
        for (int k = 0; k < 3; ++k)
        {
            node.lo[k] = llo[3 * leaf + k];
            node.hi[k] = lhi[3 * leaf + k];
        }
        node.leaf = leaf;
    }
    const int firstNode = __builtin_amdgcn_readfirstlane(t);
    const bool uniform = __builtin_amdgcn_ballot_w64(!open || t != firstNode) == 0ull;
    float lo[3], hi[3], c[3];
    if (open)
    {
        const int leaf = order[i];
        for (int k = 0; k < 3; ++k)
        {
            lo[k] = llo[3 * leaf + k];
            hi[k] = lhi[3 * leaf + k];
            c[k] = 0.5f * (lo[k] + hi[k]);
        }
    }
    if (uniform)
    {
        Node &node = nodes[firstNode];
        for (int k = 0; k < 3; ++k)
        {
            const float a = waveMin(lo[k]), b = waveMax(hi[k]), d = waveMin(c[k]), e = waveMax(c[k]);
            if ((threadIdx.x & 63) == 0)
            {
                atomicMinF(&node.lo[k], a);
                atomicMaxF(&node.hi[k], b);
                atomicMinF(&node.clo[k], d);
                atomicMaxF(&node.chi[k], e);
            }
        }
    }
    else if (open)
    {
        Node &node = nodes[t];
        for (int k = 0; k < 3; ++k)
        {
            atomicMinF(&node.lo[k], lo[k]);
            atomicMaxF(&node.hi[k], hi[k]);
            atomicMinF(&node.clo[k], c[k]);
            atomicMaxF(&node.chi[k], c[k]);
        }
    }
}

__device__ inline int binOf(float c, float origin, float scale)
{
    return min(BINS - 1, max(0, (int)((c - origin) * scale)));
}

__device__ inline void ldsMinF(float *addr, float v)
{
    v += 0.f;
    if (v >= 0.f)
        atomicMin((int *)addr, __float_as_int(v));
    else
        atomicMax((unsigned *)addr, __float_as_uint(v));
}
__device__ inline void ldsMaxF(float *addr, float v)
{
    v += 0.f;
    if (v >= 0.f)
        atomicMax((int *)addr, __float_as_int(v));
    else
        atomicMin((unsigned *)addr, __float_as_uint(v));
}

__global__ __launch_bounds__(256) void k_bins(const Node *nodes, BinSet *bins, const int *nodeOf, const int *order, const float *llo,
                                               const float *lhi, int nbLeaves, int levelFirst)
{
    __shared__ BinSet local;
    __shared__ int sameNode;
    const int i = blockIdx.x * blockDim.x + threadIdx.x;
    const int t = i < nbLeaves ? nodeOf[i] : -1;
    const bool open = t >= levelFirst && nodes[t].to - nodes[t].from > 1;
    if (threadIdx.x == 0)
        sameNode = t;
    __syncthreads();
    const int blockNode = sameNode;
    __syncthreads();
    if (!open || t != blockNode)
        sameNode = -1;
    __syncthreads();
    const bool together = sameNode >= 0;
    if (together)
    {
        for (int q = threadIdx.x; q < 3 * BINS; q += blockDim.x)
        {
            const int axis = q / BINS, bin = q % BINS;
            local.count[axis][bin] = 0;
            for (int k = 0; k < 3; ++k)
            {
                local.lo[axis][bin][k] = 1e30f;
                local.hi[axis][bin][k] = -1e30f;
            }
        }
        __syncthreads();
    }
    if (open)
    {
        const Node &node = nodes[t];
        BinSet &b = together ? local : bins[t - levelFirst];
        const int leaf = order[i];
        float lo[3], hi[3];
        for (int k = 0; k < 3; ++k)
        {
            lo[k] = llo[3 * leaf + k];
            hi[k] = lhi[3 * leaf + k];
        }
        for (int axis = 0; axis < 3; ++axis)
        {
            const float extent = node.chi[axis] - node.clo[axis];
            const float scale = extent > 0.f ? BINS / extent : 0.f;
            if (!(scale > 0.f))
                continue;
            const float c = 0.5f * (lo[axis] + hi[axis]);
            const int bin = binOf(c, node.clo[axis], scale);
            atomicAdd(&b.count[axis][bin], 1);
            for (int k = 0; k < 3; ++k)
            {
                if (together)
                {
                    ldsMinF(&b.lo[axis][bin][k], lo[k]);
                    ldsMaxF(&b.hi[axis][bin][k], hi[k]);
                }
                else
                {
                    atomicMinF(&b.lo[axis][bin][k], lo[k]);
                    atomicMaxF(&b.hi[axis][bin][k], hi[k]);
                }
            }
        }
    }
    if (together)
    {
        __syncthreads();
        BinSet &out = bins[blockNode - levelFirst];
        for (int q = threadIdx.x; q < 3 * BINS; q += blockDim.x)
        {
            const int axis = q / BINS, bin = q % BINS;
            if (local.count[axis][bin] == 0)
                continue;
            atomicAdd(&out.count[axis][bin], local.count[axis][bin]);
            for (int k = 0; k < 3; ++k)
            {
                atomicMinF(&out.lo[axis][bin][k], local.lo[axis][bin][k]);
                atomicMaxF(&out.hi[axis][bin][k], local.hi[axis][bin][k]);
            }
        }
    }
}

__device__ inline double areaOf(const float *lo, const float *hi)
{
    const double x = (double)hi[0] - lo[0], y = (double)hi[1] - lo[1], z = (double)hi[2] - lo[2];
    return x * y + y * z + z * x;
}

__global__ void k_split(Node *nodes, const BinSet *bins, int levelFirst, int count, int nextFree, int *splitting)
{
    const int i = blockIdx.x * blockDim.x + threadIdx.x;
    if (i >= count)
        return;
    Node &t = nodes[levelFirst + i];
    const int n = t.to - t.from;
    if (n < 2)
        return;
    const BinSet &b = bins[i];
    int bestAxis = -1, bestBin = 0;
    double bestCost = 1e300;
    for (int axis = 0; axis < 3; ++axis)
    {
        const float extent = t.chi[axis] - t.clo[axis];
        const float scale = extent > 0.f ? BINS / extent : 0.f;
        if (!(scale > 0.f))
            continue;
        double rightArea[BINS];
        int rightCount[BINS];
        float rlo[3] = {1e30f, 1e30f, 1e30f}, rhi[3] = {-1e30f, -1e30f, -1e30f};
        int rc = 0;
        for (int bin = BINS - 1; bin > 0; --bin)
        {
            rc += b.count[axis][bin];
            for (int k = 0; k < 3; ++k)
            {
                rlo[k] = fminf(rlo[k], b.lo[axis][bin][k]);
                rhi[k] = fmaxf(rhi[k], b.hi[axis][bin][k]);
            }
            rightCount[bin] = rc;
            rightArea[bin] = rc ? areaOf(rlo, rhi) : 0.0;
        }
        float llo[3] = {1e30f, 1e30f, 1e30f}, lhi[3] = {-1e30f, -1e30f, -1e30f};
        int lc = 0;
        for (int bin = 0; bin + 1 < BINS; ++bin)
        {
            lc += b.count[axis][bin];
            for (int k = 0; k < 3; ++k)
            {
                llo[k] = fminf(llo[k], b.lo[axis][bin][k]);
                lhi[k] = fmaxf(lhi[k], b.hi[axis][bin][k]);
            }
            if (lc == 0 || rightCount[bin + 1] == 0)
                continue;
            const double cost = areaOf(llo, lhi) * lc + rightArea[bin + 1] * rightCount[bin + 1];
            if (cost < bestCost)
            {
                bestCost = cost;
                bestAxis = axis;
                bestBin = bin;
            }
        }
    }
    t.split = 1;
    if (bestAxis < 0)
    {
        t.axis = 0;
        t.bin = -1;
        t.mid = t.from + n / 2;
    }
    else
    {
        int lc = 0;
        for (int bin = 0; bin <= bestBin; ++bin)
            lc += b.count[bestAxis][bin];
        t.axis = bestAxis;
        t.bin = bestBin;
        t.mid = t.from + lc;
    }
    const int left = nextFree + 2 * atomicAdd(splitting, 1);
    t.left = left;
    t.right = left + 1;
    nodes[left].from = t.from;
    nodes[left].to = t.mid;
    nodes[left + 1].from = t.mid;
    nodes[left + 1].to = t.to;
}

__global__ void k_flags(const Node *nodes, const int *nodeOf, const int *order, const float *llo, const float *lhi, int *flags,
                        int nbLeaves, int levelFirst)
{
    const int i = blockIdx.x * blockDim.x + threadIdx.x;
    if (i >= nbLeaves)
        return;
    const int t = nodeOf[i];
    int f = 0;
    if (t >= levelFirst && nodes[t].split)
    {
        const Node &node = nodes[t];
        if (node.bin < 0)
            f = i < node.mid;
        else
        {
            const int leaf = order[i];
            const int axis = node.axis;
            const float scale = BINS / (node.chi[axis] - node.clo[axis]);
            const float c = 0.5f * (llo[3 * leaf + axis] + lhi[3 * leaf + axis]);
            f = binOf(c, node.clo[axis], scale) <= node.bin;
        }
    }
    flags[i] = f;
}

__global__ void k_scatter(const Node *nodes, const int *nodeOf, const int *order, const int *flags, const int *before,
                          int *nodeOfOut, int *orderOut, int nbLeaves, int levelFirst)
{
    const int i = blockIdx.x * blockDim.x + threadIdx.x;
    if (i >= nbLeaves)
        return;
    const int t = nodeOf[i];
    if (t < levelFirst || !nodes[t].split)
    {
        nodeOfOut[i] = t;
        orderOut[i] = order[i];
        return;
    }
    const Node &node = nodes[t];
    const int leftRank = before[i] - before[node.from];
    const int to = flags[i] ? node.from + leftRank : node.mid + (i - node.from - leftRank);
    nodeOfOut[to] = flags[i] ? node.left : node.right;
    orderOut[to] = order[i];
}

__global__ __launch_bounds__(256) void k_prune(Node *nodes, const int *order, const float *llo, const float *lhi, int levelFirst,
                                                int count, double threshold, int nbLeaves, int *nbPruned)
{
    const int t = levelFirst + blockIdx.x;
    if ((int)blockIdx.x >= count)
        return;
    Node &node = nodes[t];
    __shared__ int inside, sampled;
    if (node.leaf >= 0)
        return;
    const int ancestor = node.keptAncestor;
    const int parentFrom = ancestor < 0 ? 0 : nodes[ancestor].from, parentTo = ancestor < 0 ? nbLeaves : nodes[ancestor].to;
    if (threadIdx.x == 0)
        inside = sampled = 0;
    __syncthreads();
    const int stride = max(1, (parentTo - parentFrom) / 4096);
    int mine = 0, seen = 0;
    for (int q = parentFrom + (int)threadIdx.x * stride; q < parentTo; q += (int)blockDim.x * stride)
    {
        const int leaf = order[q];
        bool in = true;
        for (int k = 0; k < 3 && in; ++k)
        {
            const double c = 0.5 * ((double)llo[3 * leaf + k] + lhi[3 * leaf + k]);
            in = c >= node.lo[k] && c <= node.hi[k];
        }
        ++seen;
        mine += in ? 1 : 0;
    }
    atomicAdd(&inside, mine);
    atomicAdd(&sampled, seen);
    __syncthreads();
    if (threadIdx.x != 0)
        return;
    const double parentArea = ancestor < 0 ? areaOf(nodes[0].lo, nodes[0].hi) : areaOf(nodes[ancestor].lo, nodes[ancestor].hi);
    const double bySurface = parentArea > 0.0 ? fmin(1.0, areaOf(node.lo, node.hi) / parentArea) : 1.0;
    const double byOrigin = sampled ? (double)inside / sampled : 1.0;
    const int below = 2 * (node.to - node.from) - 2;
    const bool prune = (1.0 - fmax(bySurface, byOrigin)) * below < threshold;
    node.keep = prune ? 0 : 1;
    if (prune)
        atomicAdd(nbPruned, 1);
    const int mineOrAbove = prune ? ancestor : t;
    nodes[node.left].keptAncestor = mineOrAbove;
    nodes[node.right].keptAncestor = mineOrAbove;
}

__global__ void k_sizes(Node *nodes, int levelFirst, int count)
{
    const int i = blockIdx.x * blockDim.x + threadIdx.x;
    if (i >= count)
        return;
    Node &t = nodes[levelFirst + i];
    t.size = t.leaf >= 0 ? 1 : (t.keep ? 1 : 0) + nodes[t.left].size + nodes[t.right].size;
}

__global__ void k_places(const Node *nodes, int *place, int levelFirst, int count)
{
    const int i = blockIdx.x * blockDim.x + threadIdx.x;
    if (i >= count * 8)
        return;
    const int t = levelFirst + i / 8, octant = i % 8;
    const Node &node = nodes[t];
    if (node.leaf >= 0)
        return;
    const int at = place[8 * t + octant] + (node.keep ? 1 : 0);
    const bool highFirst = (octant >> node.axis) & 1;
    const int first = highFirst ? node.right : node.left, second = highFirst ? node.left : node.right;
    place[8 * first + octant] = at;
    place[8 * second + octant] = at + nodes[first].size;
}

__global__ void k_emit(const Node *nodes, const int *place, const float4 *leafRows, const int *leafStart, const int *leafOrigin,
                       float4 *outRows, int *outStart, int *outOrigin, int nbNodes, int listLength)
{
    const int i = blockIdx.x * blockDim.x + threadIdx.x;
    if (i >= nbNodes * 8)
        return;
    const int t = i / 8, octant = i % 8;
    const Node &node = nodes[t];
    const int at = place[8 * t + octant];
    float4 *rows = outRows + 2 * (size_t)octant * listLength;
    if (node.leaf >= 0)
    {
        rows[2 * at] = leafRows[2 * node.leaf];
        float4 second = leafRows[2 * node.leaf + 1];
        second.w = __int_as_float(1);
        rows[2 * at + 1] = second;
        outStart[(size_t)octant * listLength + at] = leafStart[node.leaf];
        outOrigin[(size_t)octant * listLength + at] = leafOrigin[node.leaf];
        return;
    }
    if (!node.keep)
        return;
    rows[2 * at] = make_float4(node.lo[0], node.lo[1], node.lo[2], node.hi[2]);
    rows[2 * at + 1] = make_float4(node.hi[0], node.hi[1], __int_as_float(0), __int_as_float(node.size));
    outStart[(size_t)octant * listLength + at] = 0;
    outOrigin[(size_t)octant * listLength + at] = -1;
}

__global__ void k_iota(int *a, int n, int value, bool counting)
{
    const int i = blockIdx.x * blockDim.x + threadIdx.x;
    if (i < n)
        a[i] = counting ? i : value;
}

__global__ void k_leafFlags(const float4 *rows, int n, int *flags)
{
    const int i = blockIdx.x * blockDim.x + threadIdx.x;
    if (i <= n)
        flags[i] = i < n && __float_as_int(rows[2 * i + 1].z) > 0 ? 1 : 0;
}
__global__ void k_leafGather(const float4 *rows, const int *start, const int *before, int n, float *lo, float *hi, float4 *leafRows,
                             int *leafStart, int *leafOrigin)
{
    const int i = blockIdx.x * blockDim.x + threadIdx.x;
    if (i >= n)
        return;
    const float4 a = rows[2 * i], b = rows[2 * i + 1];
    if (__float_as_int(b.z) <= 0)
        return;
    const int l = before[i];
    lo[3 * l] = a.x, lo[3 * l + 1] = a.y, lo[3 * l + 2] = a.z;
    hi[3 * l] = b.x, hi[3 * l + 1] = b.y, hi[3 * l + 2] = a.w;
    leafRows[2 * l] = a;
    leafRows[2 * l + 1] = b;
    leafStart[l] = start[i];
    leafOrigin[l] = i;
}

inline dim3 blocksFor(size_t n, int block = 256)
{
    return dim3((unsigned)((n + block - 1) / block));
}
}

int solrBuildOrderFreeListsOnDevice(const float4 *rows, const int *start, const int *origin, int n, double threshold,
                                    int *nbPruned, hipStream_t stream, SolrDeviceLists *stay)
{
    *nbPruned = 0;
    Phase phase;
    SolrScratchPool &pool = solrScratchPool();
    std::lock_guard<std::mutex> oneBuild(pool.busy);
    struct Scope
    {
        SolrScratchPool &pool;
        ~Scope() { pool.end(); }
    } scope{pool};
    pool.begin((size_t)n * 12 + (size_t)n / 4 * (160 + 2 * sizeof(Node) + sizeof(BinSet) + 64 * sizeof(int)) + ((size_t)4 << 20));
#define LISTS_CHECK(call)                                                                                              \
    do                                                                                                                 \
    {                                                                                                                  \
        if ((call) != hipSuccess)                                                                                      \
        {                                                                                                              \
            fprintf(stderr, "solr_lists: %s failed\n", #call);                                                         \
            return -1;                                                                                                 \
        }                                                                                                              \
    } while (0)
    std::vector<float> llo, lhi;
    std::vector<float4> leafRows;
    std::vector<int> leafStart, leafOrigin;
    Dev<int> dLeafFlags, dLeafBefore;
    Dev<char> dLeafTemp;
    int L = 0;
    if (origin == nullptr)
    {
        size_t bytes = 0;
        if (!dLeafFlags.alloc((size_t)n + 1) || !dLeafBefore.alloc((size_t)n + 1))
            return -1;
        (void)hipcub::DeviceScan::ExclusiveSum(nullptr, bytes, dLeafFlags.p, dLeafBefore.p, n + 1, stream);
        if (!dLeafTemp.alloc(bytes + 256))
            return -1;
        hipLaunchKernelGGL(k_leafFlags, blocksFor((size_t)n + 1), dim3(256), 0, stream, rows, n, dLeafFlags.p);
        LISTS_CHECK(hipcub::DeviceScan::ExclusiveSum(dLeafTemp.p, bytes, dLeafFlags.p, dLeafBefore.p, n + 1, stream));
        LISTS_CHECK(hipMemcpyAsync(&L, dLeafBefore.p + n, 4, hipMemcpyDeviceToHost, stream));
        LISTS_CHECK(hipStreamSynchronize(stream));
    }
    else
    {
        for (int i = 0; i < n; ++i)
        {
            int count;
            memcpy(&count, &rows[2 * i + 1].z, 4);
            if (count <= 0)
                continue;
            llo.insert(llo.end(), {rows[2 * i].x, rows[2 * i].y, rows[2 * i].z});
            lhi.insert(lhi.end(), {rows[2 * i + 1].x, rows[2 * i + 1].y, rows[2 * i].w});
            leafRows.push_back(rows[2 * i]);
            leafRows.push_back(rows[2 * i + 1]);
            leafStart.push_back(start[i]);
            leafOrigin.push_back(origin[i]);
        }
        L = (int)leafStart.size();
    }
    if (L < 2)
        return -1;
    phase.mark("leaves gathered", L);
    const int maxNodes = 2 * L - 1;
    Dev<float> dLo, dHi;
    Dev<float4> dLeafRows, dOutRows;
    Dev<int> dLeafStart, dLeafOrigin, dOrder[2], dNodeOf[2], dFlags, dBefore, dPlace, dOutStart, dOutOrigin, dPruned;
    Dev<Node> dNodes;
    Dev<BinSet> dBins;
    Dev<char> dTemp;
    if (!dLo.alloc(3 * (size_t)L) || !dHi.alloc(3 * (size_t)L) || !dLeafRows.alloc(2 * (size_t)L) || !dLeafStart.alloc(L) ||
        !dLeafOrigin.alloc(L) || !dOrder[0].alloc(L) || !dOrder[1].alloc(L) || !dNodeOf[0].alloc(L) || !dNodeOf[1].alloc(L) ||
        !dFlags.alloc((size_t)L + 1) || !dBefore.alloc((size_t)L + 1) || !dNodes.alloc(maxNodes) ||
        !dBins.alloc(L) || !dPlace.alloc(8 * (size_t)maxNodes) || !dPruned.alloc(2))
        return -1;
    size_t tempBytes = 0;
    (void)hipcub::DeviceScan::ExclusiveSum(nullptr, tempBytes, dFlags.p, dBefore.p, L + 1, stream);
    if (!dTemp.alloc(tempBytes + 256))
        return -1;
    phase.mark("allocations");
    if (origin == nullptr)
        hipLaunchKernelGGL(k_leafGather, blocksFor(n), dim3(256), 0, stream, rows, start, dLeafBefore.p, n, dLo.p, dHi.p, dLeafRows.p,
                           dLeafStart.p, dLeafOrigin.p);
    else
    {
        LISTS_CHECK(hipMemcpyAsync(dLo.p, llo.data(), llo.size() * 4, hipMemcpyHostToDevice, stream));
        LISTS_CHECK(hipMemcpyAsync(dHi.p, lhi.data(), lhi.size() * 4, hipMemcpyHostToDevice, stream));
        LISTS_CHECK(hipMemcpyAsync(dLeafRows.p, leafRows.data(), leafRows.size() * 16, hipMemcpyHostToDevice, stream));
        LISTS_CHECK(hipMemcpyAsync(dLeafStart.p, leafStart.data(), (size_t)L * 4, hipMemcpyHostToDevice, stream));
        LISTS_CHECK(hipMemcpyAsync(dLeafOrigin.p, leafOrigin.data(), (size_t)L * 4, hipMemcpyHostToDevice, stream));
    }
    LISTS_CHECK(hipMemsetAsync(dPruned.p, 0, 4, stream));
    hipLaunchKernelGGL(k_iota, blocksFor(L), dim3(256), 0, stream, dOrder[0].p, L, 0, true);
    hipLaunchKernelGGL(k_iota, blocksFor(L), dim3(256), 0, stream, dNodeOf[0].p, L, 0, false);
    Node root;
    memset(&root, 0, sizeof(root));
    root.from = 0;
    root.to = L;
    root.keptAncestor = -1;
    LISTS_CHECK(hipMemcpyAsync(dNodes.p, &root, sizeof(root), hipMemcpyHostToDevice, stream));

    std::vector<int> levelFirst, levelCount;
    int first = 0, count = 1, nextFree = 1, cur = 0;
    for (int depth = 0; count > 0; ++depth)
    {
        if (depth >= MAX_DEPTH)
            return -1;
        levelFirst.push_back(first);
        levelCount.push_back(count);
        hipLaunchKernelGGL(k_open, blocksFor(count, 64), dim3(64), 0, stream, dNodes.p, dBins.p, first, count);
        hipLaunchKernelGGL(k_bounds, blocksFor(L), dim3(256), 0, stream, dNodes.p, dNodeOf[cur].p, dOrder[cur].p, dLo.p, dHi.p, L, first);
        hipLaunchKernelGGL(k_bins, blocksFor(L), dim3(256), 0, stream, dNodes.p, dBins.p, dNodeOf[cur].p, dOrder[cur].p, dLo.p, dHi.p, L, first);
        LISTS_CHECK(hipMemsetAsync(dPruned.p + 1, 0, 4, stream));
        hipLaunchKernelGGL(k_split, blocksFor(count, 64), dim3(64), 0, stream, dNodes.p, dBins.p, first, count, nextFree, dPruned.p + 1);
        int splitting = 0;
        LISTS_CHECK(hipMemcpyAsync(&splitting, dPruned.p + 1, 4, hipMemcpyDeviceToHost, stream));
        LISTS_CHECK(hipStreamSynchronize(stream));
        if (splitting == 0)
            break;
        if (nextFree + 2 * splitting > maxNodes)
            return -1;
        hipLaunchKernelGGL(k_flags, blocksFor(L), dim3(256), 0, stream, dNodes.p, dNodeOf[cur].p, dOrder[cur].p, dLo.p, dHi.p, dFlags.p, L, first);
        LISTS_CHECK(hipcub::DeviceScan::ExclusiveSum(dTemp.p, tempBytes, dFlags.p, dBefore.p, L + 1, stream));
        hipLaunchKernelGGL(k_scatter, blocksFor(L), dim3(256), 0, stream, dNodes.p, dNodeOf[cur].p, dOrder[cur].p, dFlags.p, dBefore.p,
                           dNodeOf[cur ^ 1].p, dOrder[cur ^ 1].p, L, first);
        cur ^= 1;
        first = nextFree;
        count = 2 * splitting;
        nextFree += count;
    }
    const int nbNodes = nextFree;
    const int levels = (int)levelFirst.size();
    phase.mark("tree, level by level", levels);
    for (int d = 0; d < levels; ++d)
        hipLaunchKernelGGL(k_prune, dim3((unsigned)levelCount[d]), dim3(256), 0, stream, dNodes.p, dOrder[cur].p, dLo.p, dHi.p, levelFirst[d],
                           levelCount[d], threshold, L, dPruned.p);
    for (int d = levels - 1; d >= 0; --d)
        hipLaunchKernelGGL(k_sizes, blocksFor(levelCount[d]), dim3(256), 0, stream, dNodes.p, levelFirst[d], levelCount[d]);
    LISTS_CHECK(hipMemsetAsync(dPlace.p, 0, 8 * sizeof(int), stream));
    for (int d = 0; d < levels; ++d)
        hipLaunchKernelGGL(k_places, blocksFor((size_t)levelCount[d] * 8), dim3(256), 0, stream, dNodes.p, dPlace.p, levelFirst[d], levelCount[d]);
    Node rootNow;
    LISTS_CHECK(hipMemcpyAsync(&rootNow, dNodes.p, sizeof(Node), hipMemcpyDeviceToHost, stream));
    LISTS_CHECK(hipMemcpyAsync(nbPruned, dPruned.p, 4, hipMemcpyDeviceToHost, stream));
    LISTS_CHECK(hipStreamSynchronize(stream));
    const int listLength = rootNow.size;
    phase.mark("pruning, sizes, places", listLength);
    if (listLength < 2)
        return -1;
    if (!dOutRows.allocOwn(16 * (size_t)listLength) || !dOutStart.allocOwn(8 * (size_t)listLength) ||
        !dOutOrigin.allocOwn(8 * (size_t)listLength))
        return -1;
    hipLaunchKernelGGL(k_emit, blocksFor((size_t)nbNodes * 8), dim3(256), 0, stream, dNodes.p, dPlace.p, dLeafRows.p, dLeafStart.p, dLeafOrigin.p,
                       dOutRows.p, dOutStart.p, dOutOrigin.p, nbNodes, listLength);
    LISTS_CHECK(hipGetLastError());
    LISTS_CHECK(hipStreamSynchronize(stream));
#undef LISTS_CHECK
    stay->rows = dOutRows.p, stay->start = dOutStart.p, stay->origin = dOutOrigin.p;
    dOutRows.p = nullptr, dOutStart.p = nullptr, dOutOrigin.p = nullptr;
    phase.mark("lists written");
    return listLength;
}


namespace
{
__global__ void k_leafCentres(const float4 *rows, const int *leaves, int nbLeaves, double *centres)
{
    const int q = blockIdx.x * blockDim.x + threadIdx.x;
    if (q >= nbLeaves)
        return;
    const int leaf = leaves[q];
    const float4 la = rows[2 * leaf], lb = rows[2 * leaf + 1];
    centres[3 * (size_t)q] = 0.5 * ((double)la.x + lb.x);
    centres[3 * (size_t)q + 1] = 0.5 * ((double)la.y + lb.y);
    centres[3 * (size_t)q + 2] = 0.5 * ((double)la.z + la.w);
}

__global__ void k_strayChildren(const float4 *rows, const int *parent, int n, char *stray)
{
    const int j = blockIdx.x * blockDim.x + threadIdx.x;
    if (j >= n || parent[j] < 0)
        return;
    const int i = parent[j];
    const float4 a = rows[2 * i], b = rows[2 * i + 1], ca = rows[2 * j], cb = rows[2 * j + 1];
    if (!(ca.x >= a.x && ca.y >= a.y && ca.z >= a.z && cb.x <= b.x && cb.y <= b.y && ca.w <= a.w))
        stray[i] = 1;
}

__global__ __launch_bounds__(256) void k_pruneList(const float4 *rows, const int *parent, const int *nodesOfDepth, int count,
                                                    const int *leavesBefore, const int *leaves, int n, double threshold,
                                                    double sceneArea, char *keep, int *keptAncestor, const char *stray, const double *centres)
{
    if ((int)blockIdx.x >= count)
        return;
    const int i = nodesOfDepth[blockIdx.x];
    __shared__ int inside, sampled, outside;
    const float4 a = rows[2 * i], b = rows[2 * i + 1];
    const int skip = max(__float_as_int(b.w), 1);
    const int end = min(i + skip, n);
    const int up = parent[i];
    const int ancestor = up < 0 ? -1 : (keep[up] ? up : keptAncestor[up]);
    if (threadIdx.x == 0)
    {
        keptAncestor[i] = ancestor;
        inside = sampled = outside = 0;
    }
    if (__float_as_int(b.z) != 0 || end <= i + 1)
        return;
    __syncthreads();
    const float lo[3] = {a.x, a.y, a.z}, hi[3] = {b.x, b.y, a.w};
    int parentFrom = 0, parentTo = n;
    double parentArea = sceneArea;
    if (ancestor >= 0)
    {
        const float4 pa = rows[2 * ancestor], pb = rows[2 * ancestor + 1];
        parentFrom = ancestor;
        parentTo = min(ancestor + max(__float_as_int(pb.w), 1), n);
        const float plo[3] = {pa.x, pa.y, pa.z}, phi[3] = {pb.x, pb.y, pa.w};
        parentArea = areaOf(plo, phi);
    }
    const int firstLeaf = leavesBefore[parentFrom], lastLeaf = leavesBefore[parentTo];
    const int stride = max(1, (lastLeaf - firstLeaf) / 4096);
    int mine = 0, seen = 0;
    for (int q = firstLeaf + (int)threadIdx.x * stride; q < lastLeaf; q += (int)blockDim.x * stride)
    {
        const double cx = centres[3 * (size_t)q], cy = centres[3 * (size_t)q + 1], cz = centres[3 * (size_t)q + 2];
        const bool in = cx >= lo[0] && cx <= hi[0] && cy >= lo[1] && cy <= hi[1] && cz >= lo[2] && cz <= hi[2];
        ++seen;
        mine += in ? 1 : 0;
    }
    const int bad = stray[i];
    atomicAdd(&inside, mine);
    atomicAdd(&sampled, seen);
    if (bad && threadIdx.x == 0)
        atomicAdd(&outside, 1);
    __syncthreads();
    if (threadIdx.x != 0)
        return;
    const double bySurface = parentArea > 0.0 ? fmin(1.0, areaOf(lo, hi) / parentArea) : 1.0;
    const double byOrigin = sampled ? (double)inside / sampled : 1.0;
    if (!outside && (1.0 - fmax(bySurface, byOrigin)) * (end - i - 1) < threshold)
        keep[i] = 0;
}
}

int solrPruneDecisionsOnDevice(const float4 *rows, int n, double threshold, std::vector<char> &keepOut, hipStream_t stream)
{
    if (n < 2)
        return -1;
    Phase phase;
    SolrScratchPool &pool = solrScratchPool();
    std::lock_guard<std::mutex> oneBuild(pool.busy);
    struct Scope
    {
        SolrScratchPool &pool;
        ~Scope() { pool.end(); }
    } scope{pool};
    pool.begin((size_t)n * 80 + ((size_t)1 << 20));
    std::vector<int> parent(n, -1), depth(n, 0), leaves, leavesBefore((size_t)n + 1, 0), stack;
    int deepest = 0;
    double sceneLo[3] = {1e300, 1e300, 1e300}, sceneHi[3] = {-1e300, -1e300, -1e300};
    auto skipOf = [&](int i) {
        int s;
        memcpy(&s, &rows[2 * i + 1].w, 4);
        return std::max(s, 1);
    };
    for (int i = 0; i < n; ++i)
    {
        while (!stack.empty() && i >= stack.back() + skipOf(stack.back()))
            stack.pop_back();
        parent[i] = stack.empty() ? -1 : stack.back();
        depth[i] = stack.empty() ? 0 : depth[stack.back()] + 1;
        deepest = std::max(deepest, depth[i]);
        stack.push_back(i);
        int count;
        memcpy(&count, &rows[2 * i + 1].z, 4);
        leavesBefore[(size_t)i + 1] = leavesBefore[i] + (count > 0 ? 1 : 0);
        if (count > 0)
            leaves.push_back(i);
        if (parent[i] < 0)
        {
            const float lo[3] = {rows[2 * i].x, rows[2 * i].y, rows[2 * i].z}, hi[3] = {rows[2 * i + 1].x, rows[2 * i + 1].y, rows[2 * i].w};
            for (int k = 0; k < 3; ++k)
            {
                sceneLo[k] = std::min(sceneLo[k], (double)lo[k]);
                sceneHi[k] = std::max(sceneHi[k], (double)hi[k]);
            }
        }
    }
    if (deepest > 256 || leaves.empty())
        return -1;
    const double sceneArea = (sceneHi[0] - sceneLo[0]) * (sceneHi[1] - sceneLo[1]) + (sceneHi[1] - sceneLo[1]) * (sceneHi[2] - sceneLo[2]) +
                             (sceneHi[2] - sceneLo[2]) * (sceneHi[0] - sceneLo[0]);
    std::vector<int> firstOfDepth((size_t)deepest + 2, 0), byDepth(n);
    for (int i = 0; i < n; ++i)
        ++firstOfDepth[(size_t)depth[i] + 1];
    for (int d = 0; d <= deepest; ++d)
        firstOfDepth[(size_t)d + 1] += firstOfDepth[d];
    {
        std::vector<int> at(firstOfDepth.begin(), firstOfDepth.end() - 1);
        for (int i = 0; i < n; ++i)
            byDepth[at[depth[i]]++] = i;
    }
    phase.mark("prune: parents and depths", deepest + 1);
    Dev<float4> dRows;
    Dev<int> dParent, dByDepth, dLeavesBefore, dLeaves, dAncestor;
    Dev<char> dKeep, dStray;
    Dev<double> dCentres;
    if (!dCentres.alloc(3 * leaves.size()) || !dStray.alloc(n) || !dRows.alloc(2 * (size_t)n) || !dParent.alloc(n) || !dByDepth.alloc(n) || !dLeavesBefore.alloc((size_t)n + 1) ||
        !dLeaves.alloc(leaves.size()) || !dAncestor.alloc(n) || !dKeep.alloc(n))
        return -1;
    bool fine = hipMemcpyAsync(dRows.p, rows, 2 * (size_t)n * 16, hipMemcpyHostToDevice, stream) == hipSuccess &&
                hipMemcpyAsync(dParent.p, parent.data(), (size_t)n * 4, hipMemcpyHostToDevice, stream) == hipSuccess &&
                hipMemcpyAsync(dByDepth.p, byDepth.data(), (size_t)n * 4, hipMemcpyHostToDevice, stream) == hipSuccess &&
                hipMemcpyAsync(dLeavesBefore.p, leavesBefore.data(), ((size_t)n + 1) * 4, hipMemcpyHostToDevice, stream) == hipSuccess &&
                hipMemcpyAsync(dLeaves.p, leaves.data(), leaves.size() * 4, hipMemcpyHostToDevice, stream) == hipSuccess &&
                hipMemsetAsync(dKeep.p, 1, n, stream) == hipSuccess && hipMemsetAsync(dStray.p, 0, n, stream) == hipSuccess;
    if (!fine)
        return -1;
    hipLaunchKernelGGL(k_strayChildren, blocksFor(n), dim3(256), 0, stream, dRows.p, dParent.p, n, dStray.p);
    hipLaunchKernelGGL(k_leafCentres, blocksFor(leaves.size()), dim3(256), 0, stream, dRows.p, dLeaves.p, (int)leaves.size(), dCentres.p);
    for (int d = 0; d <= deepest; ++d)
    {
        const int count = firstOfDepth[(size_t)d + 1] - firstOfDepth[d];
        if (count > 0)
            hipLaunchKernelGGL(k_pruneList, dim3((unsigned)count), dim3(256), 0, stream, dRows.p, dParent.p, dByDepth.p + firstOfDepth[d], count,
                               dLeavesBefore.p, dLeaves.p, n, threshold, sceneArea, dKeep.p, dAncestor.p, dStray.p, dCentres.p);
    }
    keepOut.assign(n, 1);
    if (hipMemcpyAsync(keepOut.data(), dKeep.p, n, hipMemcpyDeviceToHost, stream) != hipSuccess || hipStreamSynchronize(stream) != hipSuccess)
        return -1;
    phase.mark("prune: decisions");
    int pruned = 0;
    for (char k : keepOut)
        pruned += k ? 0 : 1;
    return pruned;
}
```

Before: 30140 Mrays/s.

## Build order-free BVH from tight plane bounds and isolate dominant leaves

The order-free list builder, on both host and device paths, now computes tight per-leaf bounds from plane primitives (with a small margin) and uses them for binning and splits. When one leaf's area dominates a node, that leaf is split off on its own along its farthest axis. Emitted inner nodes still carry the union of the uploaded leaf boxes, so the boxes used for traversal stay conservative. The aim is a tree shape that culls better for large planes like Cornell walls, at the cost of more build kernels and an extra host sync.

```diff
diff --git a/sol-r_amd/csrc/build_bounds.h b/sol-r_amd/csrc/build_bounds.h
--- /dev/null
+++ b/sol-r_amd/csrc/build_bounds.h
@@ -0,0 +1,74 @@
+#ifndef SOLR_BUILD_BOUNDS_H
+#define SOLR_BUILD_BOUNDS_H
+
+#include <hip/hip_vector_types.h>
+
+#include <cmath>
+#include <cstring>
+
+#include "../../include/solr_types.h"
+
+#if defined(__HIPCC__)
+#define SOLR_BUILD_BOUNDS_FN __host__ __device__ inline
+#else
+#define SOLR_BUILD_BOUNDS_FN inline
+#endif
+
+namespace solreng
+{
+#define SOLR_DOMINANT_SHARE 0.25
+
+struct BuildBounds
+{
+    const float4 *prims = nullptr;
+    float margin = 0.f;
+    double dominantShare = SOLR_DOMINANT_SHARE;
+};
+
+enum BuildBoundsPlainKind
+{
+    BB_KIND_SHIFT = 24,
+    BB_KIND_PLANE_XY = 2,
+    BB_KIND_PLANE_YZ = 3,
+    BB_KIND_PLANE_XZ = 4
+};
+
+SOLR_BUILD_BOUNDS_FN bool leafBuildBounds(const float4 &row0, const float4 &row1, const float4 *prims, int start, int count, float margin,
+                                          float lo[3], float hi[3], bool byKind = false)
+{
+    lo[0] = row0.x, lo[1] = row0.y, lo[2] = row0.z;
+    hi[0] = row1.x, hi[1] = row1.y, hi[2] = row0.w;
+    if (prims == nullptr || count <= 0 || start < 0)
+        return false;
+    float lx = INFINITY, ly = INFINITY, lz = INFINITY, hx = -INFINITY, hy = -INFINITY, hz = -INFINITY;
+    for (int k = 0; k < count; ++k)
+    {
+        const float4 p = prims[8 * (size_t)(start + k)], s = prims[8 * (size_t)(start + k) + 1];
+        int word;
+        memcpy(&word, &p.w, 4);
+        const int type = word & 0xff, kind = (word >> BB_KIND_SHIFT) & 15;
+        const int across = byKind ? (kind == BB_KIND_PLANE_YZ ? 0 : kind == BB_KIND_PLANE_XZ ? 1 : kind == BB_KIND_PLANE_XY ? 2 : -1)
+                                  : (type == ptYZPlane ? 0 : type == ptXZPlane ? 1 : type == ptXYPlane ? 2 : -1);
+        if (across < 0)
+            return false;
+        const float ex = across == 0 ? margin : fabsf(s.x) + margin;
+        const float ey = across == 1 ? margin : fabsf(s.y) + margin;
+        const float ez = across == 2 ? margin : fabsf(s.z) + margin;
+        lx = fminf(lx, p.x - ex), hx = fmaxf(hx, p.x + ex);
+        ly = fminf(ly, p.y - ey), hy = fmaxf(hy, p.y + ey);
+        lz = fminf(lz, p.z - ez), hz = fmaxf(hz, p.z + ez);
+    }
+    if (!(lx <= hx && ly <= hy && lz <= hz && fabsf(lx) < 3.0e38f && fabsf(hx) < 3.0e38f && fabsf(ly) < 3.0e38f && fabsf(hy) < 3.0e38f &&
+          fabsf(lz) < 3.0e38f && fabsf(hz) < 3.0e38f))
+        return false;
+    const float nlx = fmaxf(lo[0], lx), nly = fmaxf(lo[1], ly), nlz = fmaxf(lo[2], lz);
+    const float nhx = fminf(hi[0], hx), nhy = fminf(hi[1], hy), nhz = fminf(hi[2], hz);
+    if (!(nlx <= nhx && nly <= nhy && nlz <= nhz))
+        return false;
+    lo[0] = nlx, lo[1] = nly, lo[2] = nlz;
+    hi[0] = nhx, hi[1] = nhy, hi[2] = nhz;
+    return true;
+}
+}
+
+#endif
diff --git a/sol-r_amd/csrc/engine.h b/sol-r_amd/csrc/engine.h
--- a/sol-r_amd/csrc/engine.h
+++ b/sol-r_amd/csrc/engine.h
@@ -219,7 +219,8 @@
     VARIANT_NO_BAND_WORDS = 13,
     VARIANT_ZERO_STREAM_COUNTERS = 14,
     VARIANT_NO_LAMP_CUTOFF = 15,
-    VARIANT_ALL_TRIPS = 16
+    VARIANT_ALL_TRIPS = 16,
+    VARIANT_UPLOADED_BUILD_BOXES = 17
 };
 
 struct NodeList
@@ -333,6 +334,11 @@
     }
     bool orderFreeDue() { return lists.freeCountdown > 0 && --lists.freeCountdown == 0; }
     void orderFreeAskAgain() { lists.freeCountdown = 1; }
+    void orderFreeBuildAgain()
+    {
+        if (orderFree.nb > 0 && lists.freeCountdown == 0)
+            lists.freeCountdown = 1;
+    }
     void orderFreeBuilt(const NodeList &built, bool stayed, bool fromArena)
     {
         orderFree = built;
diff --git a/sol-r_amd/csrc/list_builders.cpp b/sol-r_amd/csrc/list_builders.cpp
--- a/sol-r_amd/csrc/list_builders.cpp
+++ b/sol-r_amd/csrc/list_builders.cpp
@@ -374,27 +374,31 @@
 
 int buildFreeOrderLists(const std::vector<float4> &rows, const std::vector<int> &start, const std::vector<int> &origin,
                         std::vector<float4> &outRows, std::vector<int> &outStart, std::vector<int> &outOrigin, int *nbPruned,
-                        double threshold, const PruneDecider &decider)
+                        double threshold, const PruneDecider &decider, const BuildBounds &build)
 {
     struct Leaf
     {
         float lo[3], hi[3];
         int node;
+        bool thin;
     };
     struct TreeNode
     {
         float lo[3], hi[3];
+        float ulo[3], uhi[3];
         int left, right, axis, leaf;
-        bool keep;
-    };
+        bool keep, apart;
+    };
+    bool onBuildBounds = false;
     const int n = (int)start.size();
     std::vector<Leaf> leaves;
     for (int i = 0; i < n; ++i)
         if (bitsi(rows[2 * i + 1].z) > 0)
         {
             Leaf l;
-            l.lo[0] = rows[2 * i].x, l.lo[1] = rows[2 * i].y, l.lo[2] = rows[2 * i].z;
-            l.hi[0] = rows[2 * i + 1].x, l.hi[1] = rows[2 * i + 1].y, l.hi[2] = rows[2 * i].w;
+            l.thin = leafBuildBounds(rows[2 * i], rows[2 * i + 1], build.prims, start[i], bitsi(rows[2 * i + 1].z), build.margin, l.lo, l.hi);
+            if (l.thin)
+                onBuildBounds = true;
             l.node = i;
             leaves.push_back(l);
         }
@@ -427,6 +431,7 @@
         t.axis = 0;
         t.leaf = -1;
         t.keep = true;
+        t.apart = false;
         if (count == 1)
         {
             for (int k = 0; k < 3; ++k)
@@ -449,6 +454,44 @@
             }
         for (int k = 0; k < 3; ++k)
             t.lo[k] += 0.f, t.hi[k] += 0.f;
+        if (onBuildBounds && build.dominantShare > 0.0 && count >= 3)
+        {
+            int largest = -1;
+            double largestArea = 0.0;
+            for (int q = r.from; q < r.to; ++q)
+            {
+                const double a = area(leaves[q].lo, leaves[q].hi);
+                if (a > largestArea)
+                    largestArea = a, largest = q;
+            }
+            if (largest >= 0 && largestArea > build.dominantShare * area(t.lo, t.hi))
+            {
+                const Leaf l = leaves[largest];
+                float farthest = -1.f;
+                bool lowSide = true;
+                for (int k = 0; k < 3; ++k)
+                {
+                    const float cl = 0.5f * (l.lo[k] + l.hi[k]), cu = 0.5f * (t.lo[k] + t.hi[k]);
+                    if (fabsf(cl - cu) > farthest)
+                        farthest = fabsf(cl - cu), t.axis = k, lowSide = cl <= cu;
+                }
+                if (lowSide)
+                    std::rotate(leaves.begin() + r.from, leaves.begin() + largest, leaves.begin() + largest + 1);
+                else
+                    std::rotate(leaves.begin() + largest, leaves.begin() + largest + 1, leaves.begin() + r.to);
+                const int mid = lowSide ? r.from + 1 : r.to - 1;
+                t.apart = true;
+                t.keep = false;
+                t.left = (int)tree.size();
+                t.right = t.left + 1;
+                tree.push_back(TreeNode());
+                tree.push_back(TreeNode());
+                tree[r.node] = t;
+                todo.push_back({r.from, mid, t.left});
+                todo.push_back({mid, r.to, t.right});
+                continue;
+            }
+        }
         const int BINS = 16;
         int bestAxis = -1, bestBin = 0;
         double bestCost = 1e300;
@@ -550,6 +593,28 @@
         todo.push_back({mid, r.to, t.right});
     }
 
+    for (int t = (int)tree.size() - 1; t >= 0; --t)
+    {
+        TreeNode &node = tree[t];
+        if (!onBuildBounds)
+        {
+            for (int k = 0; k < 3; ++k)
+                node.ulo[k] = node.lo[k], node.uhi[k] = node.hi[k];
+            continue;
+        }
+        if (node.leaf >= 0)
+        {
+            node.ulo[0] = rows[2 * node.leaf].x, node.ulo[1] = rows[2 * node.leaf].y, node.ulo[2] = rows[2 * node.leaf].z;
+            node.uhi[0] = rows[2 * node.leaf + 1].x, node.uhi[1] = rows[2 * node.leaf + 1].y, node.uhi[2] = rows[2 * node.leaf].w;
+            continue;
+        }
+        for (int k = 0; k < 3; ++k)
+        {
+            node.ulo[k] = std::min(tree[node.left].ulo[k], tree[node.right].ulo[k]) + 0.f;
+            node.uhi[k] = std::max(tree[node.left].uhi[k], tree[node.right].uhi[k]) + 0.f;
+        }
+    }
+
     auto flatten = [&](int octant, std::vector<float4> &fr, std::vector<int> &fs, std::vector<int> *which,
                        std::vector<int> *from) {
         struct Visit
@@ -570,9 +635,14 @@
             const TreeNode &t = tree[v.node];
             if (t.leaf >= 0)
             {
-                fr.push_back(rows[2 * t.leaf]);
-                float4 second = rows[2 * t.leaf + 1];
+                float4 first = rows[2 * t.leaf], second = rows[2 * t.leaf + 1];
+                if (onBuildBounds)
+                {
+                    first = make_float4(t.lo[0], t.lo[1], t.lo[2], t.hi[2]);
+                    second.x = t.hi[0], second.y = t.hi[1];
+                }
                 second.w = bitsf(1);
+                fr.push_back(first);
                 fr.push_back(second);
                 fs.push_back(start[t.leaf]);
                 if (which)
@@ -609,7 +679,7 @@
             kept[t] = 1;
         for (size_t t = 0; t < tree.size(); ++t)
             if (tree[t].leaf < 0)
-                tree[t].keep = kept[t] != 0;
+                tree[t].keep = kept[t] != 0 && !tree[t].apart;
     }
     std::vector<int> size(tree.size(), 0);
     for (int t = (int)tree.size() - 1; t >= 0; --t)
@@ -647,8 +717,8 @@
             int at = v.at;
             if (t.keep)
             {
-                fr[2 * at] = make_float4(t.lo[0], t.lo[1], t.lo[2], t.hi[2]);
-                fr[2 * at + 1] = make_float4(t.hi[0], t.hi[1], bitsf(0), bitsf(size[v.node]));
+                fr[2 * at] = make_float4(t.ulo[0], t.ulo[1], t.ulo[2], t.uhi[2]);
+                fr[2 * at + 1] = make_float4(t.uhi[0], t.uhi[1], bitsf(0), bitsf(size[v.node]));
                 ++at;
             }
             const bool highFirst = (octant >> t.axis) & 1;
diff --git a/sol-r_amd/csrc/list_builders.h b/sol-r_amd/csrc/list_builders.h
--- a/sol-r_amd/csrc/list_builders.h
+++ b/sol-r_amd/csrc/list_builders.h
@@ -8,6 +8,7 @@
 #include <vector>
 
 #include "../../include/solr_types.h"
+#include "build_bounds.h"
 
 namespace solreng
 {
@@ -54,7 +55,7 @@
                        const std::function<void(const char *)> &mark = nullptr);
 int buildFreeOrderLists(const std::vector<float4> &rows, const std::vector<int> &start, const std::vector<int> &origin,
                         std::vector<float4> &outRows, std::vector<int> &outStart, std::vector<int> &outOrigin, int *nbPruned,
-                        double threshold, const PruneDecider &decider = nullptr);
+                        double threshold, const PruneDecider &decider = nullptr, const BuildBounds &build = BuildBounds());
 bool listEnclosesOnHost(const std::vector<float4> &rows, const std::vector<int> &start, const std::vector<float4> &prims);
 void planRefit(const std::vector<float4> &exact, const std::vector<float4> &walk, const std::vector<int> &origin,
                const std::vector<float4> &free, const std::vector<int> &freeOrigin, std::vector<int> &plan,
diff --git a/sol-r_amd/csrc/lists_device.h b/sol-r_amd/csrc/lists_device.h
--- a/sol-r_amd/csrc/lists_device.h
+++ b/sol-r_amd/csrc/lists_device.h
@@ -2,6 +2,8 @@
 #include <hip/hip_runtime.h>
 
 #include <vector>
+
+#include "build_bounds.h"
 
 struct SolrDeviceLists
 {
@@ -11,6 +13,7 @@
 };
 
 int solrBuildOrderFreeListsOnDevice(const float4 *rows, const int *start, const int *origin, int n, double threshold,
-                                    int *nbPruned, hipStream_t stream, SolrDeviceLists *stay);
+                                    int *nbPruned, hipStream_t stream, SolrDeviceLists *stay,
+                                    const solreng::BuildBounds &build = solreng::BuildBounds());
 
 int solrPruneDecisionsOnDevice(const float4 *rows, int n, double threshold, std::vector<char> &keep, hipStream_t stream);
diff --git a/sol-r_amd/csrc/solr_arena.hip b/sol-r_amd/csrc/solr_arena.hip
--- a/sol-r_amd/csrc/solr_arena.hip
+++ b/sol-r_amd/csrc/solr_arena.hip
@@ -55,33 +55,15 @@
     const int nb = __float_as_int(row1.z);
     if (nb > 0)
     {
+        static_assert(BB_KIND_SHIFT == PRIM_KIND_SHIFT && BB_KIND_PLANE_XY == KIND_PLANE_XY && BB_KIND_PLANE_YZ == KIND_PLANE_YZ &&
+                          BB_KIND_PLANE_XZ == KIND_PLANE_XZ && ROW_P0_TYPE == 0 && ROW_SIZE_MAT == 1,
+                      "build_bounds.h reads the primitive records as scene_layout.h lays them out");
         const int start = ((const int *)arena)[offStart + (unsigned)i];
-        float lx = INFINITY, ly = INFINITY, lz = INFINITY, hx = -INFINITY, hy = -INFINITY, hz = -INFINITY;
-        bool plain = true;
-        for (int k = 0; k < nb && plain; ++k)
-        {
-            const float4 *prim = arena + offPrims + 8u * (unsigned)(start + k);
-            const float4 p = prim[ROW_P0_TYPE], s = prim[ROW_SIZE_MAT];
-            const int kind = (__float_as_int(p.w) >> PRIM_KIND_SHIFT) & 15;
-            plain = kind == KIND_PLANE_XY || kind == KIND_PLANE_YZ || kind == KIND_PLANE_XZ;
-            const float ex = kind == KIND_PLANE_YZ ? margin : fabsf(s.x) + margin;
-            const float ey = kind == KIND_PLANE_XZ ? margin : fabsf(s.y) + margin;
-            const float ez = kind == KIND_PLANE_XY ? margin : fabsf(s.z) + margin;
-            lx = fminf(lx, p.x - ex), hx = fmaxf(hx, p.x + ex);
-            ly = fminf(ly, p.y - ey), hy = fmaxf(hy, p.y + ey);
-            lz = fminf(lz, p.z - ez), hz = fmaxf(hz, p.z + ez);
-        }
-        plain = plain && lx <= hx && ly <= hy && lz <= hz && fabsf(lx) < 3.0e38f && fabsf(hx) < 3.0e38f && fabsf(ly) < 3.0e38f &&
-                fabsf(hy) < 3.0e38f && fabsf(lz) < 3.0e38f && fabsf(hz) < 3.0e38f;
-        if (plain)
-        {
-            const float nlx = fmaxf(row0.x, lx), nly = fmaxf(row0.y, ly), nlz = fmaxf(row0.z, lz);
-            const float nhx = fminf(row1.x, hx), nhy = fminf(row1.y, hy), nhz = fminf(row0.w, hz);
-            if (nlx <= nhx && nly <= nhy && nlz <= nhz)
-            {
-                row0 = make_float4(nlx, nly, nlz, nhz);
-                row1 = make_float4(nhx, nhy, row1.z, row1.w);
-            }
+        float lo[3], hi[3];
+        if (leafBuildBounds(row0, row1, arena + offPrims, start, nb, margin, lo, hi, true))
+        {
+            row0 = make_float4(lo[0], lo[1], lo[2], hi[2]);
+            row1 = make_float4(hi[0], hi[1], row1.z, row1.w);
         }
     }
     arena[offTight + 2u * (unsigned)i] = row0;
@@ -484,6 +466,12 @@
             origin[i] = i;
     };
     int prunedFree = 0;
+    BuildBounds build;
+    if (g.variant != VARIANT_UPLOADED_BUILD_BOXES)
+    {
+        build.prims = g.scene.hostPrims.data();
+        build.margin = g.facts.sceneExtent * (1.f / 1024.f);
+    }
     int count = -1;
     if (!onHost)
     {
@@ -492,13 +480,18 @@
         {
             g.scene.lists.dropStage(true);
             if (fromArena)
+            {
+                BuildBounds inArena = build;
+                if (build.prims)
+                    inArena.prims = arena + g.scene.arena.offPrims;
                 count = solrBuildOrderFreeListsOnDevice(arena + g.scene.exact.offRows, (const int *)arena + g.scene.exact.offStart, nullptr, n,
-                                                        knobs.pruneThreshold, &prunedFree, sceneStream(), &g.scene.lists.freeStage);
+                                                        knobs.pruneThreshold, &prunedFree, sceneStream(), &g.scene.lists.freeStage, inArena);
+            }
             else
             {
                 ownOrigins();
                 count = solrBuildOrderFreeListsOnDevice(rows.data(), start.data(), origin.data(), n, knobs.pruneThreshold, &prunedFree,
-                                                        sceneStream(), &g.scene.lists.freeStage);
+                                                        sceneStream(), &g.scene.lists.freeStage, build);
             }
         }
     }
@@ -509,7 +502,7 @@
         if (origin.empty())
             ownOrigins();
         count = buildFreeOrderLists(rows, start, origin, built.rows, built.start, built.origin, &prunedFree, knobs.pruneThreshold,
-                                    pruneDecider());
+                                    pruneDecider(), build);
     }
     if (getenv("SOLR_HIP_DEBUG_TREE"))
         fprintf(stderr, "solr_hip: order-free lists: 8 x %d nodes (%d inner nodes that hardly cull left out)\n", count, prunedFree);
diff --git a/sol-r_amd/csrc/solr_diag.hip b/sol-r_amd/csrc/solr_diag.hip
--- a/sol-r_amd/csrc/solr_diag.hip
+++ b/sol-r_amd/csrc/solr_diag.hip
@@ -495,6 +495,8 @@
 void solr_hip_set_variant(int variant)
 {
     onEveryDevice([&](int) {
+        if ((g.variant == VARIANT_UPLOADED_BUILD_BOXES) != (variant == VARIANT_UPLOADED_BUILD_BOXES))
+            g.scene.orderFreeBuildAgain();
         g.variant = variant;
         g.grouping = (variant != VARIANT_NO_GROUPING);
     });
diff --git a/sol-r_amd/csrc/solr_lists.hip b/sol-r_amd/csrc/solr_lists.hip
--- a/sol-r_amd/csrc/solr_lists.hip
+++ b/sol-r_amd/csrc/solr_lists.hip
@@ -46,6 +46,11 @@
     int size;
     int mid;
     int split;
+    float ulo[3], uhi[3];
+    unsigned long long largestArea;
+    int largestAt;
+    int apart;
+    int apartLeaf, lowSide;
 };
 
 struct BinSet
@@ -126,6 +131,11 @@
     t.keep = 1;
     t.split = 0;
     t.mid = t.from;
+    t.largestArea = 0ull;
+    t.largestAt = 0x7fffffff;
+    t.apart = 0;
+    t.apartLeaf = -1;
+    t.lowSide = 0;
 }
 
 __device__ inline float waveMin(float v)
@@ -312,7 +322,25 @@
     return x * y + y * z + z * x;
 }
 
-__global__ void k_split(Node *nodes, const BinSet *bins, int levelFirst, int count, int nextFree, int *splitting)
+__global__ __launch_bounds__(256) void k_largest(Node *nodes, const int *nodeOf, const int *order, const float *llo, const float *lhi,
+                                                  int nbLeaves, int levelFirst, int pass)
+{
+    const int i = blockIdx.x * blockDim.x + threadIdx.x;
+    if (i >= nbLeaves)
+        return;
+    const int t = nodeOf[i];
+    if (t < levelFirst || nodes[t].to - nodes[t].from < 3)
+        return;
+    const int leaf = order[i];
+    const unsigned long long bits = (unsigned long long)__double_as_longlong(areaOf(llo + 3 * leaf, lhi + 3 * leaf));
+    if (pass == 0)
+        atomicMax(&nodes[t].largestArea, bits);
+    else if (bits == nodes[t].largestArea)
+        atomicMin(&nodes[t].largestAt, i);
+}
+
+__global__ void k_split(Node *nodes, const BinSet *bins, int levelFirst, int count, int nextFree, int *splitting, const int *order,
+                        const float *llo, const float *lhi, double share)
 {
     const int i = blockIdx.x * blockDim.x + threadIdx.x;
     if (i >= count)
@@ -321,6 +349,35 @@
     const int n = t.to - t.from;
     if (n < 2)
         return;
+    if (share > 0.0 && n >= 3 && t.largestArea != 0ull && t.largestAt < t.to &&
+        __longlong_as_double((long long)t.largestArea) > share * areaOf(t.lo, t.hi))
+    {
+        const int leaf = order[t.largestAt];
+        float farthest = -1.f;
+        int axis = 0, lowSide = 1;
+        for (int k = 0; k < 3; ++k)
+        {
+            const float cl = 0.5f * (llo[3 * leaf + k] + lhi[3 * leaf + k]), cu = 0.5f * (t.lo[k] + t.hi[k]);
+            if (fabsf(cl - cu) > farthest)
+                farthest = fabsf(cl - cu), axis = k, lowSide = cl <= cu ? 1 : 0;
+        }
+        t.split = 1;
+        t.apart = 1;
+        t.keep = 0;
+        t.axis = axis;
+        t.bin = -2;
+        t.apartLeaf = leaf;
+        t.lowSide = lowSide;
+        t.mid = lowSide ? t.from + 1 : t.to - 1;
+        const int left = nextFree + 2 * atomicAdd(splitting, 1);
+        t.left = left;
+        t.right = left + 1;
+        nodes[left].from = t.from;
+        nodes[left].to = t.mid;
+        nodes[left + 1].from = t.mid;
+        nodes[left + 1].to = t.to;
+        return;
+    }
     const BinSet &b = bins[i];
     int bestAxis = -1, bestBin = 0;
     double bestCost = 1e300;
@@ -402,7 +459,9 @@
     if (t >= levelFirst && nodes[t].split)
     {
         const Node &node = nodes[t];
-        if (node.bin < 0)
+        if (node.bin == -2)
+            f = (order[i] == node.apartLeaf) == (node.lowSide != 0);
+        else if (node.bin < 0)
             f = i < node.mid;
         else
         {
@@ -447,6 +506,16 @@
     if (node.leaf >= 0)
         return;
     const int ancestor = node.keptAncestor;
+    if (node.apart)
+    {
+        if (threadIdx.x == 0)
+        {
+            node.keep = 0;
+            nodes[node.left].keptAncestor = ancestor;
+            nodes[node.right].keptAncestor = ancestor;
+        }
+        return;
+    }
     const int parentFrom = ancestor < 0 ? 0 : nodes[ancestor].from, parentTo = ancestor < 0 ? nbLeaves : nodes[ancestor].to;
     if (threadIdx.x == 0)
         inside = sampled = 0;
@@ -473,7 +542,7 @@
     const double parentArea = ancestor < 0 ? areaOf(nodes[0].lo, nodes[0].hi) : areaOf(nodes[ancestor].lo, nodes[ancestor].hi);
     const double bySurface = parentArea > 0.0 ? fmin(1.0, areaOf(node.lo, node.hi) / parentArea) : 1.0;
     const double byOrigin = sampled ? (double)inside / sampled : 1.0;
-    const int below = 2 * (node.to - node.from) - 2;
+    const int below = node.size - 1;
     const bool prune = (1.0 - fmax(bySurface, byOrigin)) * below < threshold;
     node.keep = prune ? 0 : 1;
     if (prune)
@@ -492,6 +561,27 @@
     t.size = t.leaf >= 0 ? 1 : (t.keep ? 1 : 0) + nodes[t.left].size + nodes[t.right].size;
 }
 
+__global__ void k_unions(Node *nodes, const float4 *leafRows, int levelFirst, int count)
+{
+    const int i = blockIdx.x * blockDim.x + threadIdx.x;
+    if (i >= count)
+        return;
+    Node &t = nodes[levelFirst + i];
+    if (t.leaf >= 0)
+    {
+        const float4 a = leafRows[2 * t.leaf], b = leafRows[2 * t.leaf + 1];
+        t.ulo[0] = a.x, t.ulo[1] = a.y, t.ulo[2] = a.z;
+        t.uhi[0] = b.x, t.uhi[1] = b.y, t.uhi[2] = a.w;
+        return;
+    }
+    const Node &l = nodes[t.left], &r = nodes[t.right];
+    for (int k = 0; k < 3; ++k)
+    {
+        t.ulo[k] = fminf(l.ulo[k], r.ulo[k]) + 0.f;
+        t.uhi[k] = fmaxf(l.uhi[k], r.uhi[k]) + 0.f;
+    }
+}
+
 __global__ void k_places(const Node *nodes, int *place, int levelFirst, int count)
 {
     const int i = blockIdx.x * blockDim.x + threadIdx.x;
@@ -509,7 +599,7 @@
 }
 
 __global__ void k_emit(const Node *nodes, const int *place, const float4 *leafRows, const int *leafStart, const int *leafOrigin,
-                       float4 *outRows, int *outStart, int *outOrigin, int nbNodes, int listLength)
+                       float4 *outRows, int *outStart, int *outOrigin, int nbNodes, int listLength, int uploaded)
 {
     const int i = blockIdx.x * blockDim.x + threadIdx.x;
     if (i >= nbNodes * 8)
@@ -530,8 +620,9 @@
     }
     if (!node.keep)
         return;
-    rows[2 * at] = make_float4(node.lo[0], node.lo[1], node.lo[2], node.hi[2]);
-    rows[2 * at + 1] = make_float4(node.hi[0], node.hi[1], __int_as_float(0), __int_as_float(node.size));
+    const float *lo = uploaded ? node.ulo : node.lo, *hi = uploaded ? node.uhi : node.hi;
+    rows[2 * at] = make_float4(lo[0], lo[1], lo[2], hi[2]);
+    rows[2 * at + 1] = make_float4(hi[0], hi[1], __int_as_float(0), __int_as_float(node.size));
     outStart[(size_t)octant * listLength + at] = 0;
     outOrigin[(size_t)octant * listLength + at] = -1;
 }
@@ -550,7 +641,7 @@
         flags[i] = i < n && __float_as_int(rows[2 * i + 1].z) > 0 ? 1 : 0;
 }
 __global__ void k_leafGather(const float4 *rows, const int *start, const int *before, int n, float *lo, float *hi, float4 *leafRows,
-                             int *leafStart, int *leafOrigin)
+                             int *leafStart, int *leafOrigin, const float4 *prims, float margin, int *anyThin)
 {
     const int i = blockIdx.x * blockDim.x + threadIdx.x;
     if (i >= n)
@@ -559,8 +650,8 @@
     if (__float_as_int(b.z) <= 0)
         return;
     const int l = before[i];
-    lo[3 * l] = a.x, lo[3 * l + 1] = a.y, lo[3 * l + 2] = a.z;
-    hi[3 * l] = b.x, hi[3 * l + 1] = b.y, hi[3 * l + 2] = a.w;
+    if (solreng::leafBuildBounds(a, b, prims, start[i], __float_as_int(b.z), margin, lo + 3 * l, hi + 3 * l))
+        *anyThin = 1;
     leafRows[2 * l] = a;
     leafRows[2 * l + 1] = b;
     leafStart[l] = start[i];
@@ -574,7 +665,7 @@
 }
 
 int solrBuildOrderFreeListsOnDevice(const float4 *rows, const int *start, const int *origin, int n, double threshold,
-                                    int *nbPruned, hipStream_t stream, SolrDeviceLists *stay)
+                                    int *nbPruned, hipStream_t stream, SolrDeviceLists *stay, const solreng::BuildBounds &build)
 {
     *nbPruned = 0;
     Phase phase;
@@ -601,6 +692,7 @@
     Dev<int> dLeafFlags, dLeafBefore;
     Dev<char> dLeafTemp;
     int L = 0;
+    int anyThin = 0;
     if (origin == nullptr)
     {
         size_t bytes = 0;
@@ -622,8 +714,11 @@
             memcpy(&count, &rows[2 * i + 1].z, 4);
             if (count <= 0)
                 continue;
-            llo.insert(llo.end(), {rows[2 * i].x, rows[2 * i].y, rows[2 * i].z});
-            lhi.insert(lhi.end(), {rows[2 * i + 1].x, rows[2 * i + 1].y, rows[2 * i].w});
+            float blo[3], bhi[3];
+            if (solreng::leafBuildBounds(rows[2 * i], rows[2 * i + 1], build.prims, start[i], count, build.margin, blo, bhi))
+                anyThin = 1;
+            llo.insert(llo.end(), {blo[0], blo[1], blo[2]});
+            lhi.insert(lhi.end(), {bhi[0], bhi[1], bhi[2]});
             leafRows.push_back(rows[2 * i]);
             leafRows.push_back(rows[2 * i + 1]);
             leafStart.push_back(start[i]);
@@ -644,7 +739,7 @@
     if (!dLo.alloc(3 * (size_t)L) || !dHi.alloc(3 * (size_t)L) || !dLeafRows.alloc(2 * (size_t)L) || !dLeafStart.alloc(L) ||
         !dLeafOrigin.alloc(L) || !dOrder[0].alloc(L) || !dOrder[1].alloc(L) || !dNodeOf[0].alloc(L) || !dNodeOf[1].alloc(L) ||
         !dFlags.alloc((size_t)L + 1) || !dBefore.alloc((size_t)L + 1) || !dNodes.alloc(maxNodes) ||
-        !dBins.alloc(L) || !dPlace.alloc(8 * (size_t)maxNodes) || !dPruned.alloc(2))
+        !dBins.alloc(L) || !dPlace.alloc(8 * (size_t)maxNodes) || !dPruned.alloc(3))
         return -1;
     size_t tempBytes = 0;
     (void)hipcub::DeviceScan::ExclusiveSum(nullptr, tempBytes, dFlags.p, dBefore.p, L + 1, stream);
@@ -652,8 +747,16 @@
         return -1;
     phase.mark("allocations");
     if (origin == nullptr)
+    {
+        LISTS_CHECK(hipMemsetAsync(dPruned.p + 2, 0, 4, stream));
         hipLaunchKernelGGL(k_leafGather, blocksFor(n), dim3(256), 0, stream, rows, start, dLeafBefore.p, n, dLo.p, dHi.p, dLeafRows.p,
-                           dLeafStart.p, dLeafOrigin.p);
+                           dLeafStart.p, dLeafOrigin.p, build.prims, build.margin, dPruned.p + 2);
+        if (build.prims)
+        {
+            LISTS_CHECK(hipMemcpyAsync(&anyThin, dPruned.p + 2, 4, hipMemcpyDeviceToHost, stream));
+            LISTS_CHECK(hipStreamSynchronize(stream));
+        }
+    }
     else
     {
         LISTS_CHECK(hipMemcpyAsync(dLo.p, llo.data(), llo.size() * 4, hipMemcpyHostToDevice, stream));
@@ -662,6 +765,8 @@
         LISTS_CHECK(hipMemcpyAsync(dLeafStart.p, leafStart.data(), (size_t)L * 4, hipMemcpyHostToDevice, stream));
         LISTS_CHECK(hipMemcpyAsync(dLeafOrigin.p, leafOrigin.data(), (size_t)L * 4, hipMemcpyHostToDevice, stream));
     }
+    const bool onBuildBounds = build.prims != nullptr && anyThin != 0;
+    const double share = onBuildBounds ? build.dominantShare : 0.0;
     LISTS_CHECK(hipMemsetAsync(dPruned.p, 0, 4, stream));
     hipLaunchKernelGGL(k_iota, blocksFor(L), dim3(256), 0, stream, dOrder[0].p, L, 0, true);
     hipLaunchKernelGGL(k_iota, blocksFor(L), dim3(256), 0, stream, dNodeOf[0].p, L, 0, false);
@@ -683,8 +788,12 @@
         hipLaunchKernelGGL(k_open, blocksFor(count, 64), dim3(64), 0, stream, dNodes.p, dBins.p, first, count);
         hipLaunchKernelGGL(k_bounds, blocksFor(L), dim3(256), 0, stream, dNodes.p, dNodeOf[cur].p, dOrder[cur].p, dLo.p, dHi.p, L, first);
         hipLaunchKernelGGL(k_bins, blocksFor(L), dim3(256), 0, stream, dNodes.p, dBins.p, dNodeOf[cur].p, dOrder[cur].p, dLo.p, dHi.p, L, first);
+        if (share > 0.0)
+            for (int pass = 0; pass < 2; ++pass)
+                hipLaunchKernelGGL(k_largest, blocksFor(L), dim3(256), 0, stream, dNodes.p, dNodeOf[cur].p, dOrder[cur].p, dLo.p, dHi.p, L, first, pass);
         LISTS_CHECK(hipMemsetAsync(dPruned.p + 1, 0, 4, stream));
-        hipLaunchKernelGGL(k_split, blocksFor(count, 64), dim3(64), 0, stream, dNodes.p, dBins.p, first, count, nextFree, dPruned.p + 1);
+        hipLaunchKernelGGL(k_split, blocksFor(count, 64), dim3(64), 0, stream, dNodes.p, dBins.p, first, count, nextFree, dPruned.p + 1,
+                           dOrder[cur].p, dLo.p, dHi.p, share);
         int splitting = 0;
         LISTS_CHECK(hipMemcpyAsync(&splitting, dPruned.p + 1, 4, hipMemcpyDeviceToHost, stream));
         LISTS_CHECK(hipStreamSynchronize(stream));
@@ -704,11 +813,16 @@
     const int nbNodes = nextFree;
     const int levels = (int)levelFirst.size();
     phase.mark("tree, level by level", levels);
+    for (int d = levels - 1; d >= 0; --d)
+        hipLaunchKernelGGL(k_sizes, blocksFor(levelCount[d]), dim3(256), 0, stream, dNodes.p, levelFirst[d], levelCount[d]);
     for (int d = 0; d < levels; ++d)
         hipLaunchKernelGGL(k_prune, dim3((unsigned)levelCount[d]), dim3(256), 0, stream, dNodes.p, dOrder[cur].p, dLo.p, dHi.p, levelFirst[d],
                            levelCount[d], threshold, L, dPruned.p);
     for (int d = levels - 1; d >= 0; --d)
         hipLaunchKernelGGL(k_sizes, blocksFor(levelCount[d]), dim3(256), 0, stream, dNodes.p, levelFirst[d], levelCount[d]);
+    if (onBuildBounds)
+        for (int d = levels - 1; d >= 0; --d)
+            hipLaunchKernelGGL(k_unions, blocksFor(levelCount[d]), dim3(256), 0, stream, dNodes.p, dLeafRows.p, levelFirst[d], levelCount[d]);
     LISTS_CHECK(hipMemsetAsync(dPlace.p, 0, 8 * sizeof(int), stream));
     for (int d = 0; d < levels; ++d)
         hipLaunchKernelGGL(k_places, blocksFor((size_t)levelCount[d] * 8), dim3(256), 0, stream, dNodes.p, dPlace.p, levelFirst[d], levelCount[d]);
@@ -724,7 +838,7 @@
         !dOutOrigin.allocOwn(8 * (size_t)listLength))
         return -1;
     hipLaunchKernelGGL(k_emit, blocksFor((size_t)nbNodes * 8), dim3(256), 0, stream, dNodes.p, dPlace.p, dLeafRows.p, dLeafStart.p, dLeafOrigin.p,
-                       dOutRows.p, dOutStart.p, dOutOrigin.p, nbNodes, listLength);
+                       dOutRows.p, dOutStart.p, dOutOrigin.p, nbNodes, listLength, onBuildBounds ? 1 : 0);
     LISTS_CHECK(hipGetLastError());
     LISTS_CHECK(hipStreamSynchronize(stream));
 #undef LISTS_CHECK
```

Measured after the change: 30720 Mrays/s (median of 6 runs). 1.9% higher.
